# renyi533/euler

Measured on AMD Instinct MI355X. Metric: train samples/sec (whole node), GraphSAGE 2-hop on 100M-node synthetic graph, higher is better.
Workload: dtype bf16; 1 GPU; model=GraphSAGE supervised (2x SAGEConv mean + fc + out_fc, sigmoid CE, Adam), global_batch=1024, parallelism=dp1, num_nodes=100000000, num_edges=950851296, feature_dim=128, feature_dtype=bf16, hidden_dim=256, label_dim=64, hipgraph=True, steps_per_graph=32, impl=euler_amd.models.sage_trainer.SageTrainer (4 fused gfx950 launches per step)

## Files before the change

### euler_amd/_build.py

```python
from __future__ import annotations

import concurrent.futures as cf
import glob
import os
import subprocess
import sys
import sysconfig

ROOT = os.path.dirname(os.path.abspath(__file__))
REPO = os.path.dirname(ROOT)
BUILD = os.environ.get("EULER_AMD_BUILD_DIR", os.path.join(os.path.expanduser("~"), ".cache", "euler_amd_build"))
CSRC = os.path.join(ROOT, "csrc")
ARCH = os.environ.get("EULER_AMD_ARCH", "gfx950")

_EXT_SUFFIX = sysconfig.get_config_var("EXT_SUFFIX") or ".so"


def _log(msg: str) -> None:
    if os.environ.get("EULER_AMD_BUILD_QUIET") != "1":
        print(f"[euler_amd build] {msg}", file=sys.stderr, flush=True)


def _newest(paths) -> float:
    m = 0.0
    for p in paths:
        try:
            m = max(m, os.path.getmtime(p))
        except OSError:
            pass
    return m


def _run(cmd):
    r = subprocess.run(cmd, stdout=subprocess.PIPE, stderr=subprocess.STDOUT, text=True)
    if r.returncode != 0:
        raise RuntimeError("command failed:\n" + " ".join(cmd) + "\n" + r.stdout)
    return r.stdout


def _compile_all(jobs, max_workers):
    todo = []
    for cmd, obj, dep_m, src in jobs:
        if os.path.exists(obj) and os.path.getmtime(obj) >= max(dep_m, os.path.getmtime(src)):
            continue
        todo.append((cmd, obj, src))
    if not todo:
        return False
    with cf.ThreadPoolExecutor(max_workers=max_workers) as ex:
        futs = {ex.submit(_run, cmd): src for cmd, obj, src in todo}
        for f in cf.as_completed(futs):
            f.result()
            _log("compiled " + os.path.relpath(futs[f], REPO))
    return True


def _pybind_includes():
    import pybind11

    return [pybind11.get_include(), sysconfig.get_paths()["include"]]


ENGINE_DIRS = ["common", "graph", "index", "framework", "gql", "ops", "rpc", "pipeline", "bindings"]


def engine_sources():
    srcs = []
    for d in ENGINE_DIRS:
        srcs += sorted(glob.glob(os.path.join(CSRC, d, "*.cc")))
    return srcs


def engine_headers():
    hs = []
    for d in ENGINE_DIRS:
        hs += glob.glob(os.path.join(CSRC, d, "*.h"))
    return hs


def engine_target():
    return os.path.join(ROOT, "_engine" + _EXT_SUFFIX)


def build_engine(max_workers: int = 8, extra_flags=None) -> str:
    out = engine_target()
    objdir = os.path.join(BUILD, "engine")
    os.makedirs(objdir, exist_ok=True)
    flags = ["-O3", "-g1", "-std=c++17", "-fPIC", "-fvisibility=hidden", "-pthread",
             "-fno-omit-frame-pointer", "-Wall", "-Wno-sign-compare", "-Wno-unused-function"]
    flags += list(extra_flags or [])
    inc = ["-I" + CSRC] + ["-I" + p for p in _pybind_includes()]
    hdr_m = _newest(engine_headers() + [__file__])
    if os.path.exists(out) and os.path.getmtime(out) >= max(hdr_m, _newest(engine_sources())):
        return out
    jobs, objs = [], []
    for s in engine_sources():
        rel = os.path.relpath(s, CSRC).replace(os.sep, "_")
        o = os.path.join(objdir, rel + ".o")
        objs.append(o)
        jobs.append((["g++"] + flags + inc + ["-c", s, "-o", o], o, hdr_m, s))
    changed = _compile_all(jobs, max_workers)
    if changed or not os.path.exists(out) or os.path.getmtime(out) < _newest(objs):
        _run(["g++", "-shared", "-pthread", "-o", out] + objs)
        _log("linked " + os.path.relpath(out, REPO))
    return out


def console_target():
    return os.path.join(ROOT, "bin", "remote_console")


def build_console(max_workers: int = 8) -> str:
    build_engine(max_workers)
    out = console_target()
    objdir = os.path.join(BUILD, "engine")
    src = os.path.join(CSRC, "tools", "remote_console.cc")
    flags = ["-O2", "-std=c++17", "-pthread", "-Wall", "-Wno-sign-compare", "-I" + CSRC]
    obj = os.path.join(objdir, "tools_remote_console.cc.o")
    hdr_m = _newest(engine_headers() + [__file__])
    _compile_all([(["g++"] + flags + ["-c", src, "-o", obj], obj, hdr_m, src)], 1)
    objs = []
    for s in engine_sources():
        if os.sep + "bindings" + os.sep in s:
            continue
        o = os.path.join(objdir, os.path.relpath(s, CSRC).replace(os.sep, "_") + ".o")
        if not os.path.exists(o):
            _compile_all([(["g++", "-O3", "-std=c++17", "-fPIC", "-pthread", "-I" + CSRC] +
                           ["-I" + p for p in _pybind_includes()] + ["-c", s, "-o", o], o, hdr_m, s)], 1)
        objs.append(o)
    if not os.path.exists(out) or os.path.getmtime(out) < _newest(objs + [obj]):
        os.makedirs(os.path.dirname(out), exist_ok=True)
        _run(["g++", "-pthread", "-o", out, obj] + objs + ["-ldl"])
        _log("linked " + os.path.relpath(out, REPO))
    return out


_SANITIZERS = {
    "thread": ["-fsanitize=thread"],
    "address": ["-fsanitize=address,undefined", "-fno-sanitize-recover=undefined"],
    "none": [],
}


def build_selftest(sanitize: str = "thread", max_workers: int = 8) -> str:
    if sanitize not in _SANITIZERS:
        raise ValueError("sanitize must be one of %s" % sorted(_SANITIZERS))
    objdir = os.path.join(BUILD, "selftest_" + sanitize)
    os.makedirs(objdir, exist_ok=True)
    out = os.path.join(objdir, "engine_selftest")
    san = _SANITIZERS[sanitize]
    flags = ["-O1", "-g", "-std=c++17", "-pthread", "-fno-omit-frame-pointer", "-Wno-sign-compare"] + san
    srcs = [s for s in engine_sources() if os.sep + "bindings" + os.sep not in s]
    srcs.append(os.path.join(CSRC, "tests", "engine_selftest.cc"))
    hdr_m = _newest(engine_headers() + [__file__])
    jobs, objs = [], []
    for s in srcs:
        rel = os.path.relpath(s, CSRC).replace(os.sep, "_")
        o = os.path.join(objdir, rel + ".o")
        objs.append(o)
        jobs.append((["g++"] + flags + ["-I" + CSRC, "-c", s, "-o", o], o, hdr_m, s))
    changed = _compile_all(jobs, max_workers)
    if changed or not os.path.exists(out) or os.path.getmtime(out) < _newest(objs):
        _run(["g++"] + san + ["-pthread", "-o", out] + objs + ["-ldl"])
        _log("linked " + os.path.relpath(out, REPO))
    return out


def build_plan_selftest() -> str:
    objdir = os.path.join(BUILD, "selftest_address")
    os.makedirs(objdir, exist_ok=True)
    out = os.path.join(objdir, "tree_plan_selftest")
    src = os.path.join(CSRC, "tests", "tree_plan_selftest.cc")
    hdir = os.path.join(CSRC, "hip")
    deps = [src, os.path.join(hdir, "tree_plan.h"), os.path.join(hdir, "tree_args.h"), __file__]
    if not os.path.exists(out) or os.path.getmtime(out) < _newest(deps):
        rocm_inc = os.path.join(os.environ.get("ROCM_PATH", "/opt/rocm"), "include")
        _run(["g++", "-O1", "-g", "-std=c++17", "-fno-omit-frame-pointer", "-Wall"] + _SANITIZERS["address"] +
             ["-D__HIP_PLATFORM_AMD__=1", "-I" + CSRC, "-I" + rocm_inc, src, "-o", out])
        _log("linked " + os.path.relpath(out, REPO))
    return out


def hip_target():
    return os.path.join(ROOT, "_hip_ops" + _EXT_SUFFIX)


def _torch_paths():
    import torch

    tdir = os.path.dirname(torch.__file__)
    inc = [os.path.join(tdir, "include"), os.path.join(tdir, "include", "torch", "csrc", "api", "include")]
    return tdir, inc, os.path.join(tdir, "lib"), bool(torch._C._GLIBCXX_USE_CXX11_ABI)


def build_hip(max_workers: int = 8) -> str:
    hipcc = os.environ.get("HIPCC", "/opt/rocm/bin/hipcc")
    out = hip_target()
    objdir = os.path.join(BUILD, "hip")
    os.makedirs(objdir, exist_ok=True)
    tdir, tinc, tlib, abi = _torch_paths()
    hdir = os.path.join(CSRC, "hip")
    kernels = sorted(glob.glob(os.path.join(hdir, "*.hip")))
    bindings = sorted(glob.glob(os.path.join(hdir, "*.cpp")))
    hdrs = glob.glob(os.path.join(hdir, "*.h")) + [__file__]
    hdr_m = _newest(hdrs)
    if os.path.exists(out) and os.path.getmtime(out) >= max(hdr_m, _newest(kernels + bindings)):
        return out
    kflags = ["-O3", "-std=c++17", "-fPIC", f"--offload-arch={ARCH}", "-munsafe-fp-atomics",
              "-D__HIP_PLATFORM_AMD__=1", "-I" + CSRC, "-Wno-unused-result"]
    kflags += os.environ.get("EULER_AMD_HIP_FLAGS", "").split()
    bflags = ["-O2", "-std=c++17", "-fPIC", "-D__HIP_PLATFORM_AMD__=1", "-DUSE_ROCM=1",
              f"-D_GLIBCXX_USE_CXX11_ABI={int(abi)}", "-DTORCH_API_INCLUDE_EXTENSION_H",
              "-DTORCH_EXTENSION_NAME=_hip_ops", "-I" + CSRC, "-I/opt/rocm/include",
              "-Wno-unused-result", "-Wno-deprecated-declarations"]
    bflags += ["-I" + p for p in tinc + _pybind_includes()]
    jobs, objs = [], []
    for s in kernels:
        o = os.path.join(objdir, os.path.basename(s) + ".o")
        objs.append(o)
        jobs.append(([hipcc] + kflags + ["-c", s, "-o", o], o, hdr_m, s))
    for s in bindings:
        o = os.path.join(objdir, os.path.basename(s) + ".o")
        objs.append(o)
        jobs.append((["g++"] + bflags + ["-c", s, "-o", o], o, hdr_m, s))
    changed = _compile_all(jobs, max_workers)
    if changed or not os.path.exists(out) or os.path.getmtime(out) < _newest(objs):
        link = [hipcc, "-shared", "-fPIC", f"--offload-arch={ARCH}", "-o", out] + objs + [
            "-L" + tlib, "-Wl,-rpath," + tlib, "-lc10", "-lc10_hip", "-ltorch", "-ltorch_cpu",
            "-ltorch_hip", "-ltorch_python", "-lamdhip64"]
        _run(link)
        _log("linked " + os.path.relpath(out, REPO))
    return out


def build_all(max_workers: int = 8) -> None:
    if engine_sources():
        build_engine(max_workers)
        build_console(max_workers)
    build_hip(max_workers)


if __name__ == "__main__":
    what = sys.argv[1:] or ["all"]
    if "all" in what:
        build_all()
    else:
        if "engine" in what:
            build_engine()
        if "hip" in what:
            build_hip()
        if "console" in what:
            build_console()
```

### euler_amd/csrc/hip/binding_tree.cpp

```cpp
#include <cstdio>
#include <cstdlib>

#include "hip/binding_util.h"
#include "hip/tree_plan.h"

using namespace euler_bind;
using namespace euler_hip;

namespace {

bool sync_debug() {
  static const bool on = [] {
    const char* e = std::getenv("EULER_AMD_TREE_SYNC");
    return e && e[0] == '1';
  }();
  return on;
}

void tree_ok(hipError_t e, const char* what) {
  launch_ok(e, what);
  if (sync_debug()) {
    const hipError_t s = hipStreamSynchronize(cur_stream());
    TORCH_CHECK(s == hipSuccess, "euler_amd tree kernel '", what, "' faulted: ", hipGetErrorString(s));
    fprintf(stderr, "[tree-sync] %s ok\n", what);
  }
}

void fill_graph_tree(PlanDict& pd, TrGraph& g, TrTree& tr, int64_t F1, int64_t F2, int64_t logP1, int64_t logP2,
                     uint32_t m1, uint32_t m2) {
  torch::Tensor indptr = pd.T("indptr"), rng = pd.T("rng");
  pd.need(indptr, torch::kInt64, -1, "indptr");
  pd.need(rng, torch::kInt64, 2, "rng");
  const int64_t nt = pd.geti("num_types");
  TORCH_CHECK(nt >= 1 && nt <= 32 && (indptr.numel() - 1) % nt == 0, pd.name(), ": indptr must be [N*T+1]");
  g.indptr = indptr.data_ptr<int64_t>();
  g.num_types = static_cast<int32_t>(nt);
  g.num_rows = (indptr.numel() - 1) / nt;
  torch::Tensor nbr = pd.T("nbr"), cumw = pd.T("cumw"), prob = pd.T("node_prob");
  pd.need(nbr, torch::kInt32, -1, "nbr");
  pd.need(cumw, torch::kFloat32, nbr.numel(), "cumw");
  g.nbr = nbr.data_ptr<int32_t>();
  g.cumw = cumw.data_ptr<float>();
  pd.need(prob, torch::kFloat32, -1, "node_prob");
  g.pop = prob.numel();
  TORCH_CHECK(g.pop > 0, pd.name(), ": empty root population");
  g.prob = prob.data_ptr<float>();
  g.alias = pd.i32("node_alias", g.pop);
  g.root_rows = pd.has("root_rows") ? pd.i32("root_rows", g.pop) : nullptr;
  tr.rng = rng.data_ptr<int64_t>();
  tr.F1 = static_cast<int32_t>(F1);
  tr.F2 = static_cast<int32_t>(F2);
  tr.logP1 = static_cast<int32_t>(logP1);
  tr.logP2 = static_cast<int32_t>(logP2);
  tr.m1 = m1;
  tr.m2 = m2;
}

int plan_route_impl(const PlanDict& pd) {
  const int64_t impl = pd.has("dw_route_impl") ? pd.geti("dw_route_impl") : 2;
  TORCH_CHECK(impl == 0 || impl == 2, pd.name(), ": dw_route_impl must be 0 or 2");
  return static_cast<int>(impl);
}

bool plan_fuse_key(const PlanDict& pd) {
  const int64_t f = pd.has("dw_opt_fuse") ? pd.geti("dw_opt_fuse") : 1;
  TORCH_CHECK(f == 0 || f == 1, pd.name(), ": dw_opt_fuse must be 0 or 1");
  return f == 1;
}

class DwPlan {
 public:
  explicit DwPlan(PlanDict& pd) : pd_(pd), route_impl_(plan_route_impl(pd)), fuse_key_(plan_fuse_key(pd)) {}

  std::vector<TrDwProb> probs;
  TrOptArgs opt{};

  const TrDwProb& add(int64_t P, int64_t Q, int64_t M, const uint16_t* G, const uint16_t* X, const float* dA,
                      const uint32_t* mask, int64_t logPg, int64_t Fg, int64_t self) {
    TORCH_CHECK(M % 32 == 0 && P % 32 == 0 && Q % 32 == 0, pd_.name(), ": dW problem shapes");
    TrDwProb p{};
    p.P = static_cast<int32_t>(P);
    p.Q = static_cast<int32_t>(Q);
    p.MB = static_cast<int32_t>(M / 32);
    if (dA) {
      TORCH_CHECK(tr_plan_routed(p, pd_.has("dw_route_wg") ? pd_.geti("dw_route_wg") : 256), pd_.name(),
                  ": routed dW needs P % 64 == 0 and a positive dw_route_wg");
      p.route = 1;
      p.dA = dA;
      p.mask = mask;
      p.logPg = static_cast<int32_t>(logPg);
      p.Fg = static_cast<int32_t>(Fg);
      p.include_self = static_cast<int32_t>(self);
      p.inv = 1.f / static_cast<float>(Fg + self);
    } else {
      const int64_t target = pd_.has("dw_target_wg") ? pd_.geti("dw_target_wg") : 512;
      const int64_t minkps = pd_.has("dw_min_kps") ? pd_.geti("dw_min_kps") : 4;
      const int64_t fold = pd_.has("dw_fold") ? pd_.geti("dw_fold") : 1;
      TORCH_CHECK(target >= 1 && minkps >= 1 && (fold == 0 || fold == 1), pd_.name(),
                  ": dw_target_wg / dw_min_kps must be positive, dw_fold 0 or 1");
      tr_plan_stored(p, target, minkps, fold == 1);
    }
    p.part = pd_.zeros_ptr<float>(static_cast<int64_t>(p.S) * P * Q, torch::kFloat32);
    p.G = G;
    p.X = X;
    probs.push_back(p);
    return probs.back();
  }

  void add_seg(int64_t off, const TrDwProb& p, const uint16_t* sh, const uint16_t* shT) {
    TrSeg& g = next_seg();
    g.off = off;
    g.n = static_cast<int64_t>(p.P) * p.Q;
    g.part = p.part;
    g.S = p.S;
    g.rows = p.P;
    g.cols = p.Q;
    g.sh = const_cast<uint16_t*>(sh);
    g.shT = const_cast<uint16_t*>(shT);
  }
  void add_vec_seg(int64_t off, int64_t n, const float* part, int64_t S) {
    TrSeg& g = next_seg();
    g.off = off;
    g.n = n;
    g.part = part;
    g.S = static_cast<int32_t>(S);
    g.rows = 1;
  }
  void layout_segs() {
    opt.nblk = tr_seg_layout(opt.seg, opt.nseg, true);
    TORCH_CHECK(opt.nblk >= 1, pd_.name(), ": weight segments need rows % 8, cols % 32");
  }

  void fill_opt(int64_t n, const float* head_part, int64_t nhead, bool rank_stat) {
    torch::Tensor flat = pd_.T("flat");
    pd_.need(flat, torch::kFloat32, -1, "flat");
    const int64_t nbuf = flat.numel();
    TORCH_CHECK(n <= nbuf, pd_.name(), ": offsets must lie inside the flat buffer");
    opt.n = n;
    opt.p = flat.data_ptr<float>();
    opt.g = pd_.f32("grad", nbuf);
    opt.m = pd_.f32("m", nbuf);
    opt.v = pd_.f32("v", nbuf);
    TrOptCore& c = opt.c;
    c.step = pd_.ptr<int64_t>("step", torch::kInt64, 1);
    c.lr = static_cast<float>(pd_.getf("lr"));
    c.b1 = static_cast<float>(pd_.getf("beta1"));
    c.b2 = static_cast<float>(pd_.getf("beta2"));
    c.eps = static_cast<float>(pd_.getf("eps"));
    c.wd = static_cast<float>(pd_.getf("weight_decay"));
    c.grad_scale = 1.f;
    c.kind = static_cast<int32_t>(pd_.geti("opt_kind"));
    c.head_part = head_part;
    c.nhead = static_cast<int32_t>(nhead);
    c.loss_acc = pd_.f32("loss_acc", 1);
    c.loss_out = pd_.f32("loss_out", 1);
    if (rank_stat) c.stat_f = pd_.f32("mrr_sum", 1);
    else c.counts = reinterpret_cast<uint32_t*>(pd_.i32("counts", 3));
  }

  void try_fuse(bool allowed) {
    TrDwGrid grid;
    TrDwLaunch L = launch_of(all(), false, grid);
    if (!fuse_key_ || !allowed || !tr_dw_fuse(L, opt, fopt_)) return;
    sync_ = pd_.zeros(static_cast<int64_t>(fopt_.nsync) * kTrSyncLine, torch::kInt32);
    fopt_.sync = reinterpret_cast<uint32_t*>(sync_.data_ptr<int32_t>());
    fused_ = true;
  }
  bool fused() const { return fused_; }
  int64_t fuse_error() const { return sync_.defined() ? sync_[kTrSyncLine].item<int64_t>() : 0; }

  std::vector<int64_t> all() const {
    std::vector<int64_t> w(probs.size());
    for (size_t i = 0; i < w.size(); ++i) w[i] = static_cast<int64_t>(i);
    return w;
  }

  void launch(const std::vector<int64_t>& which, c10::optional<torch::Tensor> prof, bool fuse, double grad_scale) {
    const c10::DeviceGuard g(pd_.device());
    TrDwGrid grid;
    TrDwLaunch L = launch_of(which, fuse, grid);
    if (fuse) L.opt.c.grad_scale = static_cast<float>(grad_scale);
    if (prof.has_value()) {
      pd_.need(*prof, torch::kInt64, -1, "prof");
      L.prof = reinterpret_cast<long long*>(prof->data_ptr<int64_t>());
    }
    tree_ok(eh_tr_dw(&L, cur_stream()), fuse ? "tr_dw+opt" : "tr_dw");
  }
  int64_t blocks(const std::vector<int64_t>& which, bool fuse) const {
    TrDwGrid grid;
    launch_of(which, fuse, grid);
    return grid.ndw + grid.ntrail;
  }
  std::vector<int64_t> splits() const {
    std::vector<int64_t> s;
    for (const auto& p : probs) s.push_back(p.S);
    return s;
  }
  std::vector<int64_t> folds() const {
    std::vector<int64_t> f;
    for (const auto& p : probs) f.push_back(p.F);
    return f;
  }
  void set_lr(double lr) { opt.c.lr = fopt_.c.lr = static_cast<float>(lr); }
  void set_grad(torch::Tensor g, bool exact) {
    pd_.need(g, torch::kFloat32, exact ? opt.n : -1, "grad");
    TORCH_CHECK(g.numel() >= opt.n, "grad has ", g.numel(), " elements, fewer than the ", opt.n, " parameters");
    grad_ = g;
    opt.g = g.data_ptr<float>();
  }

 private:
  PlanDict& pd_;
  int route_impl_;
  bool fuse_key_, fused_ = false;
  TrDwOpt fopt_{};
  torch::Tensor sync_;
  torch::Tensor grad_;

  TrSeg& next_seg() {
    TORCH_CHECK(opt.nseg < kTrMaxSegs, pd_.name(), ": too many optimizer segments");
    return opt.seg[opt.nseg++] = TrSeg{};
  }

  TrDwLaunch launch_of(const std::vector<int64_t>& which, bool fuse, TrDwGrid& grid) const {
    TrDwLaunch L{};
    L.route_impl = route_impl_;
    bool every = which.size() == probs.size();
    for (size_t k = 0; k < which.size(); ++k) {
      const int64_t i = which[k];
      TORCH_CHECK(i >= 0 && i < (int64_t)probs.size(), "dw: problem index out of range");
      every = every && i == (int64_t)k;
      if (probs[i].route) {
        TORCH_CHECK(L.nroute < 2, "dw: at most two routed problems per launch");
        L.route[L.nroute++] = probs[i];
      } else {
        TORCH_CHECK(L.plain.n < kTrMaxProbs, "dw: too many problems");
        L.plain.p[L.plain.n++] = probs[i];
      }
    }
    if (fuse) {
      TORCH_CHECK(fused_ && every, pd_.name(),
                  ": the optimizer runs in the dW launch of every problem, in the plan's order, of a fused() plan only");
      L.opt = fopt_;
      L.fuse = 1;
    }
    TORCH_CHECK(tr_dw_layout(L, grid), pd_.name(), ": the dW launch is not one the kernel takes");
    return L;
  }
};

class TreePlan : private PlanDict {
 public:
  explicit TreePlan(py::dict d) : PlanDict(d, "TreePlan") {
    L_ = geti("L");
    B_ = geti("B");
    TORCH_CHECK(L_ >= 1 && L_ <= 3, "TreePlan: 1..3 hops");
    TORCH_CHECK(B_ > 0 && B_ % 32 == 0, "TreePlan: batch must be a positive multiple of 32");
    F_ = getv("F");
    logP_ = getv("logP");
    masks_ = getv("masks");
    dims_ = getv("H");
    TORCH_CHECK((int)F_.size() == L_ + 1 && (int)masks_.size() == L_ + 1 && (int)logP_.size() >= L_ &&
                    (int)dims_.size() == L_,
                "TreePlan: F/masks need L+1 entries (index 0 unused), logP L, H L");
    D_ = geti("D");
    E_ = geti("E");
    C_ = geti("C");
    C_real_ = geti("C_real");
    self_ = geti("include_self");
    for (int k = 1; k < L_; ++k) TORCH_CHECK(logP_[k] >= 4 && (1 << logP_[k]) > F_[k], "TreePlan: slot group too small");
    for (int k = 0; k < L_; ++k) TORCH_CHECK(dims_[k] % 64 == 0, "TreePlan: conv widths must be padded to 64");
    TORCH_CHECK(D_ % 16 == 0 && E_ % 32 == 0 && C_ % 32 == 0 && C_real_ <= C_, "TreePlan: padded dims");
    M_.assign(L_, 0);
    M_[0] = B_;
    for (int k = 1; k < L_; ++k) M_[k] = M_[k - 1] << logP_[k];
    fill_graph_tree(*this, graph_, tree_, L_ > 1 ? F_[1] : 0, L_ > 2 ? F_[2] : 0, L_ > 1 ? logP_[1] : 0,
                    L_ > 2 ? logP_[2] : 0, static_cast<uint32_t>(masks_[1]),
                    L_ > 2 ? static_cast<uint32_t>(masks_[2]) : 0u);
    build_fwd();
    build_comb();
    build_head();
    build_dw();
    build_opt();
    dw_.try_fuse(!pipeline_ok());
  }

  bool fused() const { return dw_.fused(); }
  int64_t fuse_error() const { return dw_.fuse_error(); }

  void sample() {
    const c10::DeviceGuard g(device());
    tree_ok(eh_tr_sample(&sample_, cur_stream()), "tr_sample");
  }

  void fwd(c10::optional<torch::Tensor> prof, bool gemm_only) {
    const c10::DeviceGuard g(device());
    TORCH_CHECK(!gemm_only || pipeline_ok(), "TreePlan: no pipelined forward for this plan");
    TrFwdArgs a0 = fwd0_;
    if (prof.has_value()) {
      need(*prof, torch::kInt64, (fwd0_.M / (gemm_only ? 64 : bm0_)) * 8, "prof");
      a0.prof = reinterpret_cast<long long*>(prof->data_ptr<int64_t>());
    }
    tree_ok(eh_tr_fwd(&a0, gemm_only ? 3 : (L_ == 1 ? 1 : 0), feat_fp32_, bm0_, cur_stream()), "tr_fwd");
    if (L_ == 3) tree_ok(eh_tr_fwd(&fwd1_, 2, 0, bm1_, cur_stream()), "tr_fwd(inner)");
  }

  void head(c10::optional<torch::Tensor> prof, bool with_sample) {
    const c10::DeviceGuard g(device());
    TrHeadArgs a = head_;
    if (with_sample) {
      a.smp = sample_;
      a.nsample = static_cast<int32_t>((sample_.M + kTrHeadSampleRows - 1) / kTrHeadSampleRows);
    }
    if (prof.has_value()) {
      need(*prof, torch::kInt64, (B_ / kTrHeadRows) * 8, "prof");
      a.prof = reinterpret_cast<long long*>(prof->data_ptr<int64_t>());
    }
    tree_ok(eh_tr_head(&a, B_, cur_stream()), "tr_head");
  }

  void bwd() {
    if (L_ != 3) return;
    const c10::DeviceGuard g(device());
    tree_ok(eh_tr_bwd(&bwd1_, cur_stream()), "tr_bwd");
  }

  void dw(std::vector<int64_t> which, c10::optional<torch::Tensor> prof, bool fuse, double grad_scale) {
    dw_.launch(which, prof, fuse, grad_scale);
  }
  int64_t dw_blocks(bool fuse) const { return dw_.blocks(dw_.all(), fuse); }

  std::vector<int64_t> problems(bool route) const {
    std::vector<int64_t> out;
    for (size_t i = 0; i < dw_.probs.size(); ++i)
      if (static_cast<bool>(dw_.probs[i].route) == route) out.push_back(static_cast<int64_t>(i));
    return out;
  }

  void opt(int64_t mode, double grad_scale, bool with_sample, bool with_gather) {
    const c10::DeviceGuard g(device());
    TORCH_CHECK(!with_gather || pipeline_ok(), "TreePlan: no pipelined gather for this plan");
    TrOptArgs a = dw_.opt;
    a.c.grad_scale = static_cast<float>(grad_scale);
    if (!with_sample) a.nsample = 0;
    if (with_gather) {
      a.gat = fwd0_;
      a.ngather = static_cast<int32_t>(fwd0_.M / 32);
      a.gat_fp32 = feat_fp32_;
      static const int first = [] {
        const char* e = std::getenv("EULER_AMD_GATHER_FIRST");
        return e ? std::atoi(e) : 1;
      }();
      a.gather_first = first;
      static const int tpb = [] {
        const char* e = std::getenv("EULER_AMD_OPT_TPB");
        return e ? std::atoi(e) : 4;
      }();
      a.opt_tpb = tpb;
    }
    tree_ok(eh_tr_opt(&a, static_cast<int>(mode), cur_stream()), "tr_opt");
  }

  bool pipeline_ok() const {
    return L_ == 2 && fwd0_.a_rows != nullptr && !cached_ && bm0_ <= 64 && logP_[1] <= 5 && D_ % 64 == 0 &&
           fwd0_.M % 64 == 0 && dims_[0] <= 256 &&
           eh_tr_gather32_lds(static_cast<int>(D_), static_cast<int>(fwd0_.FL)) <= 64 * 1024;
  }

  void opt_segments(int64_t mode, std::vector<int64_t> segs, bool head_stats) {
    TORCH_CHECK(mode == 0, "opt_segments: only the reduce (mode 0) runs on a segment subset");
    TORCH_CHECK(!segs.empty() && (int64_t)segs.size() <= dw_.opt.nseg, "opt_segments: bad segment list");
    const c10::DeviceGuard g(device());
    TrOptArgs a = dw_.opt;
    a.nseg = 0;
    for (int64_t k : segs) {
      TORCH_CHECK(k >= 0 && k < dw_.opt.nseg, "opt_segments: segment index out of range");
      a.seg[a.nseg++] = dw_.opt.seg[k];
    }
    a.nblk = tr_seg_layout(a.seg, a.nseg, true);
    a.nsample = 0;
    if (!head_stats) a.c.nhead = 0;
    tree_ok(eh_tr_opt(&a, 0, cur_stream()), "tr_opt(segments)");
  }

  int64_t fwd_blocks() const { return fwd0_.M / bm0_; }
  void set_lr(double lr) { dw_.set_lr(lr); }
  void set_grad(torch::Tensor g) { dw_.set_grad(g, true); }
  void set_grad16(c10::optional<torch::Tensor> g16) {
    if (!g16.has_value()) {
      dw_.opt.g16 = nullptr;
      g16_ = torch::Tensor();
      return;
    }
    need(*g16, torch::kBFloat16, dw_.opt.n, "grad16");
    g16_ = *g16;
    dw_.opt.g16 = reinterpret_cast<uint16_t*>(g16_.data_ptr());
  }
  int64_t num_problems() const { return (int64_t)dw_.probs.size(); }
  int64_t route_blocks(int64_t i) const { return dw_.probs.at(i).route ? dw_.blocks({i}, false) : 0; }
  std::vector<int64_t> splits() const { return dw_.splits(); }
  std::vector<int64_t> folds() const { return dw_.folds(); }

 private:
  int L_, B_, D_, E_, C_, C_real_, self_;
  int feat_fp32_ = 0, bm0_ = 32, bm1_ = 32;
  bool cached_ = false;
  std::vector<int64_t> F_, logP_, masks_, dims_, M_;
  TrGraph graph_{};
  TrTree tree_{};
  TrSampleArgs sample_{};
  TrFwdArgs fwd0_{}, fwd1_{};
  TrHeadArgs head_{};
  TrBwdArgs bwd1_{};
  DwPlan dw_{*this};
  torch::Tensor roots_cur_;
  torch::Tensor g16_;

  int64_t Hin(int k) const { return k == 0 ? D_ : dims_[k - 1]; }

  void build_fwd() {
    const bool cached = has("fwd_features");
    torch::Tensor x = cached ? T("fwd_features") : T("features");
    feat_fp32_ = !need_bf16_or_f32(x, -1, "features");
    TORCH_CHECK(x.dim() == 2 && x.size(1) == D_, "features must be [N, D] with D padded to 16");
    TORCH_CHECK(cached || x.size(0) == graph_.num_rows, "features must have one row per graph row");
    const int lv = L_ - 1;
    const int64_t M = M_[lv];
    TrSampleArgs& sm = sample_;
    sm.g = graph_;
    sm.tr = tree_;
    sm.M = M;
    sm.lv = lv;
    sm.FL = static_cast<int32_t>(F_[L_]);
    sm.mL = static_cast<uint32_t>(masks_[L_]);
    sm.hopL = L_;
    sm.roots = i32("roots", B_);
    sm.nodes = i32("nodes", M);
    sm.leaf = i32("leaf", M * sm.FL);
    TrFwdArgs& a = fwd0_;
    a.x = x.data_ptr();
    a.D = D_;
    a.M = M;
    a.FL = sm.FL;
    a.include_self = self_;
    a.inv_leaf = 1.f / static_cast<float>(a.FL + self_);
    cached_ = cached;
    a.nodes = cached ? i32("fwd_nodes", M) : sm.nodes;
    a.leaf = cached ? i32("fwd_leaf", M * sm.FL) : sm.leaf;
    a.roots_in = sm.roots;
    roots_cur_ = zeros(B_, torch::kInt32);
    a.roots_cur = roots_cur_.data_ptr<int32_t>();
    a.B = B_;
    a.step = ptr<int64_t>("step", torch::kInt64, 1);
    a.rng = ptr<int64_t>("rng", torch::kInt64, 2);
    if (L_ == 1) {
      a.a_next = bf("A0", B_ * 2 * D_);
      bm0_ = 32;
      return;
    }
    a.W = bf("W0_sh", dims_[0] * 2 * D_);
    a.H = static_cast<int32_t>(dims_[0]);
    a.a_kt = bf("A0_kt", M * 2 * D_);
    a.mask = i32_as_u32("mask0", (M / 32) * dims_[0]);
    a.logPg = static_cast<int32_t>(logP_[lv]);
    a.Fg = static_cast<int32_t>(F_[lv]);
    a.inv_grp = 1.f / static_cast<float>(a.Fg + self_);
    a.a_next = bf("A1", M_[lv - 1] * 2 * dims_[0]);
    a.a_rows = has("A0_rows") ? bf("A0_rows", M * 2 * D_) : nullptr;
    bm0_ = (1 << a.logPg) > 32 ? (1 << a.logPg) : 32;
    if (has("fwd_bm")) bm0_ = std::max<int>(bm0_, static_cast<int>(geti("fwd_bm")));
    TORCH_CHECK(bm0_ == 32 || bm0_ == 64 || bm0_ == 128, "TreePlan: fwd rows per block must be 32, 64 or 128");
    TORCH_CHECK(M % bm0_ == 0, "TreePlan: target rows must be a multiple of the fwd block rows");
    if (L_ == 3) {
      TrFwdArgs& b = fwd1_;
      b.x = T("A1").data_ptr();
      b.D = static_cast<int32_t>(dims_[0]);
      b.M = M_[1];
      b.include_self = self_;
      b.W = bf("W1_sh", dims_[1] * 2 * dims_[0]);
      b.H = static_cast<int32_t>(dims_[1]);
      b.a_kt = bf("A1_kt", M_[1] * 2 * dims_[0]);
      b.mask = i32_as_u32("mask1", (M_[1] / 32) * dims_[1]);
      b.logPg = static_cast<int32_t>(logP_[1]);
      b.Fg = static_cast<int32_t>(F_[1]);
      b.inv_grp = 1.f / static_cast<float>(b.Fg + self_);
      b.a_next = bf("A2", B_ * 2 * dims_[1]);
      bm1_ = (1 << b.logPg) > 32 ? (1 << b.logPg) : 32;
    }
  }

  void build_comb() {
    torch::Tensor flat = T("flat");
    need(flat, torch::kFloat32, -1, "flat");
    std::vector<int64_t> off = getv("offsets");
    TORCH_CHECK((int)off.size() == L_ + 4 && off.back() == flat.numel(), "TreePlan: offsets must cover the flat buffer");
    const int64_t H = dims_[L_ - 1];
    TORCH_CHECK(off[L_ + 1] - off[L_] == (int64_t)E_ * H && off[L_ + 3] - off[L_ + 2] == (int64_t)C_ * E_,
                "TreePlan: fc / out_fc segments do not match E, H, C");
    TORCH_CHECK(C_ % 16 == 0 && H % 16 == 0 && E_ % 32 == 0, "TreePlan: combination tiles need C % 16, H % 16, E % 32");
    float* base = flat.data_ptr<float>();
    TrCombArgs& c = fwd0_.comb;
    c.bfc = base + off[L_ + 1];
    c.wout = base + off[L_ + 2];
    c.wout_sh = bf("Wout_sh", (int64_t)C_ * E_);
    c.wfcT_sh = bf("Wfc_shT", (int64_t)E_ * H);
    c.C = C_;
    c.E = E_;
    c.H = static_cast<int32_t>(H);
    c.Wc = zeros_ptr<uint16_t>((int64_t)C_ * H, torch::kBFloat16);
    c.WcT = zeros_ptr<uint16_t>((int64_t)C_ * H, torch::kBFloat16);
    c.bc = zeros_ptr<float>(C_, torch::kFloat32);
    fwd0_.ncomb = 1;
  }

  uint32_t* i32_as_u32(const std::string& k, int64_t numel) { return reinterpret_cast<uint32_t*>(i32(k, numel)); }

  void build_head() {
    const int last = L_ - 1;
    const int64_t Hin2 = 2 * Hin(last), H = dims_[last];
    TrHeadArgs& a = head_;
    a.A = bf("A" + std::to_string(last), B_ * Hin2);
    a.Hin2 = static_cast<int32_t>(Hin2);
    a.H = static_cast<int32_t>(H);
    a.E = E_;
    a.C = C_;
    a.C_real = C_real_;
    a.W = bf("W" + std::to_string(last) + "_sh", H * Hin2);
    a.WT = L_ > 1 ? bf("W" + std::to_string(last) + "_shT", H * Hin2) : nullptr;
    a.Wfc = bf("Wfc_sh", (int64_t)E_ * H);
    a.WfcT = bf("Wfc_shT", (int64_t)E_ * H);
    a.Wout = bf("Wout_sh", (int64_t)C_ * E_);
    a.WoutT = bf("Wout_shT", (int64_t)C_ * E_);
    a.bfc = f32("bfc", E_);
    a.Wc = fwd0_.comb.Wc;
    a.WcT = fwd0_.comb.WcT;
    a.bc = fwd0_.comb.bc;
    a.roots = fwd0_.roots_cur;
    const int mode = static_cast<int>(geti("label_mode"));
    torch::Tensor lab = T("labels");
    need_any(lab, "labels");
    TORCH_CHECK(mode >= 0 && mode <= 2, "label_mode must be 0, 1 or 2");
    const int64_t lrows = has("label_rows") ? geti("label_rows") : graph_.num_rows;
    if (mode == 0) {
      TORCH_CHECK(lab.scalar_type() == torch::kInt16 && lab.numel() == lrows, "TreePlan: labels int16 [N]");
    } else if (mode == 1) {
      TORCH_CHECK(lab.scalar_type() == torch::kInt32 && lab.numel() == lrows, "TreePlan: labels int32 [N]");
    } else {
      TORCH_CHECK(lab.scalar_type() == torch::kBFloat16 && lab.numel() == lrows * C_, "TreePlan: labels bf16 [N, C]");
    }
    a.labels = lab.data_ptr();
    a.label_mode = mode;
    a.inv_scale = 1.f / static_cast<float>(B_ * C_real_);
    a.A_kt = bf("A" + std::to_string(last) + "_kt", B_ * Hin2);
    a.h_kt = bf("h_kt", B_ * H);
    a.emb_kt = bf("emb_kt", (int64_t)B_ * E_);
    a.dlog_kt = bf("dlog_kt", (int64_t)B_ * C_);
    a.demb_kt = bf("demb_kt", (int64_t)B_ * E_);
    a.g_kt = bf("g_kt", B_ * H);
    a.dA = L_ > 1 ? f32("dA" + std::to_string(last), B_ * Hin2) : nullptr;
    const int64_t nblk = B_ / kTrHeadRows;
    a.dbfc_part = zeros_ptr<float>(nblk * E_, torch::kFloat32);
    a.head_part = zeros_ptr<float>(nblk * 4, torch::kFloat32);
    a.prof = nullptr;
    const size_t lds = eh_tr_head_lds(a.Hin2, a.H, a.E, a.C, mode);
    TORCH_CHECK(lds <= 160 * 1024 - 64, "TreePlan: head tile does not fit in LDS (", lds, " bytes)");
    if (L_ == 3) {
      TrBwdArgs& b = bwd1_;
      b.dA = f32("dA2", B_ * 2 * dims_[1]);
      b.mask = i32_as_u32("mask1", (M_[1] / 32) * dims_[1]);
// ... 146 lines not shown
  int bm() const { return bm_; }
  int64_t R() const { return R_; }
  int64_t H() const { return H_; }
  int64_t D() const { return D_; }
  using PlanDict::device;

  void bwd() {
    dw_.launch({0}, c10::nullopt, false, 1.0);
    const c10::DeviceGuard g(device());
    tree_ok(eh_tr_opt(&dw_.opt, 0, cur_stream()), "tower reduce");
  }

 private:
  int64_t R_, F1_, F2_, logP_, D_, H_, self_, M_;
  int feat_fp32_ = 0, bm_ = 32;
  TrGraph g_{};
  TrTree tree_{};
  TrSampleArgs sample_{};
  TrFwdArgs fwd_{};
  DwPlan dw_{*this};

  int32_t* owned_i32(int64_t n) { return full(n, -1, torch::kInt32).data_ptr<int32_t>(); }
};

class PairPlan : private PlanDict {
 public:
  PairPlan(const TowerPlan& s, const TowerPlan& c, py::dict d) : PlanDict(d, "PairPlan", s.device()) {
    B_ = geti("B");
    K_ = geti("K");
    H0_ = s.H();
    H1_ = geti("H1");
    E_ = geti("E");
    TORCH_CHECK(c.R() == B_ * (1 + K_) && s.R() == B_, "PairPlan: tower roots must be B and B (1 + K)");
    TORCH_CHECK(c.H() == H0_ && c.D() == s.D(), "PairPlan: towers must have the same layer-0 shape");
    TORCH_CHECK(B_ % 32 == 0 && K_ >= 1 && K_ <= 15, "PairPlan: B % 32 == 0 and 1 <= K <= 15");
    TORCH_CHECK(H1_ % 64 == 0 && E_ % 32 == 0, "PairPlan: padded dims (H1 % 64, E % 32)");
    TORCH_CHECK(eh_tr_pair_head_lds(static_cast<int>(K_), static_cast<int>(2 * H0_), static_cast<int>(H1_),
                                    static_cast<int>(E_)) <= 160 * 1024 - 256,
                "PairPlan: the pair head does not fit in LDS (K / widths too large)");
    fpx_ = s.feat_fp32();
    bm_s_ = s.bm();
    bm_c_ = c.bm();
    ss_ = s.sample_args();
    sc_ = c.sample_args();
    ss_.tr.root_in = nullptr;
    ss_.tr.root_mode = 0;
    ss_.tr.stream_off = 0;
    sc_.tr.root_in = nullptr;
    sc_.tr.root_mode = 1;
    sc_.tr.pair_B = static_cast<int32_t>(B_);
    sc_.tr.pair_mask = static_cast<uint32_t>(geti("pos_mask"));
    sc_.tr.stream_off = 8;
    fs_ = s.fwd_args();
    fc_ = c.fwd_args();
    fs_.roots_in = ss_.roots;
    fc_.roots_in = sc_.roots;
    fs_.step = ptr<int64_t>("step", torch::kInt64, 1);
    fc_.step = nullptr;
    fc_.rng = zeros_ptr<int64_t>(2, torch::kInt64);
    nblk_ = B_ / 16;
    TrPairHeadArgs& h = head_;
    h.B = static_cast<int32_t>(B_);
    h.K = static_cast<int32_t>(K_);
    h.H0x2 = static_cast<int32_t>(2 * H0_);
    h.H1 = static_cast<int32_t>(H1_);
    h.E = static_cast<int32_t>(E_);
    h.inv_n = 1.f / static_cast<float>(B_ * (1 + K_));
    h.head_part = zeros_ptr<float>(nblk_ * 4, torch::kFloat32);
    tower(h.s, s, "s");
    tower(h.c, c, "c");
    const TowerPlan* tp[2] = {&s, &c};
    const TrPairTower* tw[2] = {&h.s, &h.c};
    for (int t = 0; t < 2; ++t) dw_.probs.push_back(tp[t]->prob());
    for (int t = 0; t < 2; ++t) {
      dw_.add(H1_, 2 * H0_, tp[t]->R(), tw[t]->g_kt, tw[t]->A1_kt, nullptr, nullptr, 0, 0, 0);
      dw_.add(E_, H1_, tp[t]->R(), tw[t]->de_kt, tw[t]->h_kt, nullptr, nullptr, 0, 0, 0);
    }
    std::vector<int64_t> off = getv("offsets");
    TORCH_CHECK(off.size() == 9, "PairPlan: offsets = 8 segments + end");
    for (int t = 0; t < 2; ++t) {
      const TrPairTower& T_ = *tw[t];
      dw_.add_seg(off[4 * t], dw_.probs[t], tp[t]->fwd_args().W, nullptr);
      dw_.add_seg(off[4 * t + 1], dw_.probs[2 + 2 * t], T_.W1, T_.W1T);
      dw_.add_seg(off[4 * t + 2], dw_.probs[3 + 2 * t], T_.Wfc, T_.WfcT);
      dw_.add_vec_seg(off[4 * t + 3], E_, T_.dbfc_part, nblk_);
      TORCH_CHECK(off[4 * t + 4] - off[4 * t + 3] == E_, "PairPlan: bias segment must be E long");
    }
    dw_.layout_segs();
    dw_.fill_opt(off.back(), h.head_part, nblk_, true);
    dw_.try_fuse(true);
  }

  bool fused() const { return dw_.fused(); }
  int64_t fuse_error() const { return dw_.fuse_error(); }

  void sample() {
    const c10::DeviceGuard g(device());
    tree_ok(eh_tr_sample(&ss_, cur_stream()), "pair sample (source)");
    tree_ok(eh_tr_sample(&sc_, cur_stream()), "pair sample (context)");
  }
  void fwd() {
    const c10::DeviceGuard g(device());
    tree_ok(eh_tr_fwd(&fs_, 0, fpx_, bm_s_, cur_stream()), "pair fwd (source)");
    tree_ok(eh_tr_fwd(&fc_, 0, fpx_, bm_c_, cur_stream()), "pair fwd (context)");
  }
  void head() {
    const c10::DeviceGuard g(device());
    tree_ok(eh_tr_pair_head(&head_, cur_stream()), "pair head");
  }
  void dw(bool fuse, double grad_scale) { dw_.launch(dw_.all(), c10::nullopt, fuse, grad_scale); }
  void opt(int mode, double grad_scale) {
    const c10::DeviceGuard g(device());
    TrOptArgs a = dw_.opt;
    a.c.grad_scale = static_cast<float>(grad_scale);
    tree_ok(eh_tr_opt(&a, mode, cur_stream()), "pair opt");
  }
  void set_lr(double lr) { dw_.set_lr(lr); }
  void set_grad(torch::Tensor g) { dw_.set_grad(g, false); }
  std::vector<int64_t> splits() const { return dw_.splits(); }
  std::vector<int64_t> folds() const { return dw_.folds(); }

 private:
  int64_t B_, K_, H0_, H1_, E_, nblk_;
  int fpx_ = 0, bm_s_ = 32, bm_c_ = 32;
  TrSampleArgs ss_{}, sc_{};
  TrFwdArgs fs_{}, fc_{};
  TrPairHeadArgs head_{};
  DwPlan dw_{*this};

  void tower(TrPairTower& t, const TowerPlan& tp, const std::string& x) {
    const int64_t R = tp.R();
    t.A1 = tp.fwd_args().a_next;
    t.W1 = bf(("W1_sh_" + x).c_str(), H1_ * 2 * H0_);
    t.W1T = bf(("W1_shT_" + x).c_str(), H1_ * 2 * H0_);
    t.Wfc = bf(("Wfc_sh_" + x).c_str(), E_ * H1_);
    t.WfcT = bf(("Wfc_shT_" + x).c_str(), E_ * H1_);
    t.bfc = ptr<float>(("bfc_" + x).c_str(), torch::kFloat32, E_);
    t.A1_kt = zeros_ptr<uint16_t>(R * 2 * H0_, torch::kBFloat16);
    t.h_kt = zeros_ptr<uint16_t>(R * H1_, torch::kBFloat16);
    t.de_kt = zeros_ptr<uint16_t>(R * E_, torch::kBFloat16);
    t.g_kt = zeros_ptr<uint16_t>(R * H1_, torch::kBFloat16);
    t.dA1 = const_cast<float*>(tp.prob().dA);
    t.dbfc_part = zeros_ptr<float>(nblk_ * E_, torch::kFloat32);
  }
};

}

void register_tree_ops(py::module& m) {
  static_assert(kTrHeadSampleRows == 256, "head sampler blocks: 1024 threads, 256 rows");
  py::class_<TreePlan>(m, "TreePlan")
      .def(py::init<py::dict>())
      .def("sample", &TreePlan::sample)
      .def("fwd", &TreePlan::fwd, py::arg("prof") = py::none(), py::arg("gemm_only") = false)
      .def("fwd_blocks", [](const TreePlan& t) { return t.fwd_blocks(); })
      .def("head", &TreePlan::head, py::arg("prof") = py::none(), py::arg("with_sample") = false)
      .def("bwd", &TreePlan::bwd)
      .def("dw", &TreePlan::dw, py::arg("which"), py::arg("prof") = py::none(), py::arg("fuse") = false,
           py::arg("grad_scale") = 1.0)
      .def("fused", &TreePlan::fused)
      .def("dw_blocks", &TreePlan::dw_blocks, py::arg("fuse"))
      .def("fuse_error", &TreePlan::fuse_error)
      .def("route_blocks", &TreePlan::route_blocks)
      .def("opt", &TreePlan::opt, py::arg("mode"), py::arg("grad_scale") = 1.0, py::arg("with_sample") = false,
           py::arg("with_gather") = false)
      .def("pipeline_ok", &TreePlan::pipeline_ok)
      .def("opt_segments", &TreePlan::opt_segments, py::arg("mode"), py::arg("segs"), py::arg("head_stats"))
      .def("set_lr", &TreePlan::set_lr)
      .def("set_grad16", &TreePlan::set_grad16, py::arg("g16"))
      .def("set_grad", &TreePlan::set_grad, py::arg("g"))
      .def("num_problems", &TreePlan::num_problems)
      .def("splits", &TreePlan::splits)
      .def("folds", &TreePlan::folds)
      .def("problems", &TreePlan::problems, py::arg("route"));
  m.attr("tree_head_rows") = kTrHeadRows;
  py::class_<TowerPlan>(m, "TowerPlan")
      .def(py::init<py::dict>())
      .def("shadow", &TowerPlan::shadow)
      .def("sample", &TowerPlan::sample)
      .def("fwd", &TowerPlan::fwd)
      .def("bwd", &TowerPlan::bwd)
      .def("fused", &TowerPlan::fused)
      .def("fuse_error", &TowerPlan::fuse_error);
  py::class_<PairPlan>(m, "PairPlan")
      .def(py::init<const TowerPlan&, const TowerPlan&, py::dict>(), py::keep_alive<1, 2>(), py::keep_alive<1, 3>())
      .def("sample", &PairPlan::sample)
      .def("fwd", &PairPlan::fwd)
      .def("head", &PairPlan::head)
      .def("dw", &PairPlan::dw, py::arg("fuse") = false, py::arg("grad_scale") = 1.0)
      .def("fused", &PairPlan::fused)
      .def("fuse_error", &PairPlan::fuse_error)
      .def("opt", &PairPlan::opt, py::arg("mode"), py::arg("grad_scale") = 1.0)
      .def("set_lr", &PairPlan::set_lr)
      .def("set_grad", &PairPlan::set_grad)
      .def("splits", &PairPlan::splits)
      .def("folds", &PairPlan::folds);
}
```

### euler_amd/csrc/hip/tree_args.h

```cpp
#pragma once
#include <hip/hip_runtime_api.h>
#include <stdint.h>

namespace euler_hip {

constexpr int kTrMaxProbs = 6;
constexpr int kTrMaxSegs = 8;
constexpr int kTrHeadRows = 16;
constexpr int kTrHeadSampleRows = 256;

struct TrGraph {
  const int64_t* indptr;
  const int32_t* nbr;
  const float* cumw;
  int64_t num_rows;
  int32_t num_types;
  const float* prob;
  const int32_t* alias;
  const int32_t* root_rows;
  int64_t pop;
};

struct TrTree {
  const int64_t* rng;
  const int32_t* root_in;
  int32_t F1, F2;
  int32_t logP1, logP2;
  uint32_t m1, m2;
  int32_t root_mode, pair_B;
  uint32_t pair_mask;
  int32_t stream_off;
};

struct TrSampleArgs {
  TrGraph g;
  TrTree tr;
  int64_t M;
  int32_t lv;
  int32_t FL;
  uint32_t mL;
  int32_t hopL;
  int32_t* roots;
  int32_t* nodes;
  int32_t* leaf;
};

struct TrCombArgs {
  const float* wout;
  const float* bfc;
  const uint16_t* wout_sh;
  const uint16_t* wfcT_sh;
  int32_t C, E, H;
  uint16_t* Wc;
  uint16_t* WcT;
  float* bc;
};

struct TrFwdArgs {
  const void* x;
  int32_t D;
  int64_t M;
  int32_t FL;
  int32_t include_self;
  float inv_leaf;
  const int32_t* nodes;
  const int32_t* leaf;
  const uint16_t* W;
  int32_t H;
  uint16_t* a_kt;
  uint32_t* mask;
  uint16_t* a_next;
  int32_t logPg, Fg;
  float inv_grp;
  int64_t* step;
  int64_t* rng;
  const int32_t* roots_in;
  int32_t* roots_cur;
  int32_t B;
  long long* prof;
  TrCombArgs comb;
  int32_t ncomb;
  uint16_t* a_rows;
};

struct TrHeadArgs {
  const uint16_t* A;
  int32_t Hin2, H, E, C, C_real;
  const uint16_t *W, *WT, *Wfc, *WfcT, *Wout, *WoutT;
  const uint16_t *Wc, *WcT;
  const float* bfc;
  const float* bc;
  const int32_t* roots;
  const void* labels;
  int32_t label_mode;
  float inv_scale;
  uint16_t *A_kt, *h_kt, *emb_kt, *dlog_kt, *demb_kt, *g_kt;
  float* dA;
  float* dbfc_part;
  float* head_part;
  long long* prof;
  TrSampleArgs smp;
  int32_t nsample;
};

struct TrPairTower {
  const uint16_t* A1;
  const uint16_t *W1, *W1T;
  const uint16_t *Wfc, *WfcT;
  const float* bfc;
  uint16_t *A1_kt, *h_kt, *de_kt, *g_kt;
  float* dA1;
  float* dbfc_part;
};
struct TrPairHeadArgs {
  TrPairTower s, c;
  int32_t B, K, H0x2, H1, E;
  float inv_n;
  float* head_part;
};

struct TrBwdArgs {
  const float* dA;
  const uint32_t* mask;
  const uint16_t* WT;
  int32_t Hk, K2out;
  int64_t M;
  int32_t logPg, Fg, include_self;
  float inv;
  float* dA_out;
};

struct TrDwProb {
  const uint16_t* G;
  const uint16_t* X;
  float* part;
  int32_t P, Q, MB, kps, S, tiles_q, ntiles, wg0;
  int32_t F;
  const float* dA;
  const uint32_t* mask;
  int32_t route, logPg, Fg, include_self;
  float inv;
};
struct TrDwProbs {
  TrDwProb p[kTrMaxProbs];
  int32_t n;
};
constexpr int kTrFoldLds = 64 * 1024;
constexpr int kTrFoldMax = kTrFoldLds / (32 * 32 * 4);

struct TrSeg {
  int64_t off, n;
  const float* part;
  int32_t S;
  int32_t rows, cols;
  int32_t blk0;
  uint16_t* sh;
  uint16_t* shT;
  int32_t sgrp;
};
struct TrOptCore {
  const int64_t* step;
  float lr, b1, b2, eps, wd, grad_scale;
  int32_t kind;
  const float* head_part;
  int32_t nhead;
  float* loss_acc;
  uint32_t* counts;
  float* loss_out;
  float* stat_f;
};
struct TrOptArgs {
  float *p, *g, *m, *v;
  uint16_t* g16;
  int64_t n;
  TrSeg seg[kTrMaxSegs];
  int32_t nseg;
  int32_t nblk;
  TrOptCore c;
  TrSampleArgs smp;
  int32_t nsample;
  TrFwdArgs gat;
  int32_t ngather;
  int32_t gat_fp32;
  int32_t gather_first;
  int32_t opt_tpb;
};

struct TrFoldSeg {
  int64_t off;
  uint16_t *sh, *shT;
};
struct TrDwOpt {
  float *p, *m, *v;
  TrSeg seg[kTrMaxSegs];
  int32_t nseg, nblk;
  int32_t rseg0;
  TrFoldSeg fseg[kTrMaxProbs];
  TrOptCore c;
  uint32_t* sync;
  int32_t nsync;
  int32_t cnt0[2];
  long long timeout;
};
constexpr int kTrSyncLine = 32;
constexpr uint32_t kTrFuseTimeout = 1u;
constexpr long long kTrFuseWaitTicks = 1200000;

struct TrDwLaunch {
  TrDwProbs plain;
  TrDwProb route[2];
  int32_t nroute;
  int32_t rwg[3];
  int32_t route_impl;
  long long* prof;
  int32_t ndw;
  int32_t fuse;
  TrDwOpt opt;
};

}

extern "C" {
hipError_t eh_tr_sample(const euler_hip::TrSampleArgs* a, hipStream_t s);
hipError_t eh_tr_fwd(const euler_hip::TrFwdArgs* a, int mode, int feat_fp32, int bm, hipStream_t s);
size_t eh_tr_gather32_lds(int D, int FL);
hipError_t eh_tr_head(const euler_hip::TrHeadArgs* a, int64_t B, hipStream_t s);
hipError_t eh_tr_bwd(const euler_hip::TrBwdArgs* a, hipStream_t s);
hipError_t eh_tr_dw(euler_hip::TrDwLaunch* p, hipStream_t s);
hipError_t eh_tr_opt(const euler_hip::TrOptArgs* a, int mode, hipStream_t s);
size_t eh_tr_fwd_lds(int D, int H, int bm, int FL, int mode);
size_t eh_tr_fwd2_lds(int D, int FL);
size_t eh_tr_head_lds(int Hin2, int H, int E, int C, int label_mode);
size_t eh_tr_pair_head_lds(int K, int H0x2, int H1, int E);
hipError_t eh_tr_pair_head(const euler_hip::TrPairHeadArgs* a, hipStream_t s);
}
```

### euler_amd/csrc/hip/tree_dev.h

```cpp
#pragma once
#include "hip/tile.h"
#include "hip/tree_args.h"

namespace euler_hip {

constexpr uint64_t kTrStreamRoot = 1, kTrStreamPos = 2, kTrStreamNeg = 3, kTrStreamHop = 16;

#define TR_STAMP(prof, blk, k) \
  if ((prof) && threadIdx.x == 0) (prof)[(blk) * 8 + (k)] = static_cast<long long>(wall_clock64())

__device__ __forceinline__ uint4_t tr_rand(const int64_t* rng, uint64_t stream, uint64_t idx) {
  return Philox::gen(static_cast<uint64_t>(rng[0]), (static_cast<uint64_t>(rng[1]) << 8) ^ stream, idx);
}

__device__ __forceinline__ int32_t tr_root(const TrGraph& g, const int64_t* rng, int64_t t,
                                           uint64_t stream = kTrStreamRoot) {
  const uint4_t r = tr_rand(rng, stream, static_cast<uint64_t>(t));
  const uint64_t x = (static_cast<uint64_t>(r[0]) << 32) | r[1];
  int64_t k = static_cast<int64_t>(__umul64hi(x, static_cast<uint64_t>(g.pop)));
  if (k >= g.pop) k = g.pop - 1;
  const int64_t pick = (u01(r[2]) < g.prob[k]) ? k : static_cast<int64_t>(g.alias[k]);
  return g.root_rows ? g.root_rows[pick] : static_cast<int32_t>(pick);
}

// ... 2 lines not shown
  const int64_t base = static_cast<int64_t>(row) * g.num_types;
  int64_t lo = 0, hi = 0;
  float total = 0.f;
  if (g.num_types == 1) {
    if (!(mask & 1u)) return -1;
    lo = g.indptr[base];
    hi = g.indptr[base + 1];
    total = hi > lo ? g.cumw[hi - 1] : 0.f;
  } else {
    float tot = 0.f;
    for (int t = 0; t < g.num_types; ++t) {
      if (!((mask >> t) & 1u)) continue;
      const int64_t a = g.indptr[base + t], b = g.indptr[base + t + 1];
      if (b > a) tot += g.cumw[b - 1];
    }
    if (!(tot > 0.f)) return -1;
    float u = u01(r[0]) * tot;
    for (int t = 0; t < g.num_types; ++t) {
      if (!((mask >> t) & 1u)) continue;
      const int64_t a = g.indptr[base + t], b = g.indptr[base + t + 1];
      if (b <= a) continue;
      const float gw = g.cumw[b - 1];
      lo = a;
      hi = b;
      total = gw;
      if (u < gw) break;
      u -= gw;
    }
  }
  if (hi <= lo || !(total > 0.f)) return -1;
  const float u = u01(r[1]) * total;
  int64_t a = lo, b = hi - 1;
  while (a < b) {
    const int64_t m = (a + b) >> 1;
    if (g.cumw[m] > u) b = m;
    else a = m + 1;
  }
  return g.nbr[a];
}

__device__ __forceinline__ int32_t tr_hop(const TrGraph& g, const int64_t* rng, int32_t parent, int j, int F,
                                          uint32_t mask, int hop, int64_t parent_slot, int stream_off = 0) {
  if (j < F)
    return parent >= 0 ? tr_neighbor(g, parent, mask,
                                     tr_rand(rng, kTrStreamHop + hop + stream_off,
                                             static_cast<uint64_t>(parent_slot * F + j)))
                       : -1;
  return j == F ? parent : -1;
}

__device__ __forceinline__ int32_t tr_tree_root(const TrGraph& g, const TrTree& tr, int64_t t) {
  if (tr.root_in) return tr.root_in[t];
  if (tr.root_mode == 0) return tr_root(g, tr.rng, t);
  if (t < tr.pair_B) {
    const int32_t src = tr_root(g, tr.rng, t);
    return src >= 0 ? tr_neighbor(g, src, tr.pair_mask, tr_rand(tr.rng, kTrStreamPos, static_cast<uint64_t>(t)))
                    : -1;
  }
  return tr_root(g, tr.rng, t, kTrStreamNeg);
}

__device__ int32_t tr_slot_node(const TrGraph& g, const TrTree& tr, int64_t s, int lv, int64_t* root,
                                bool* self_chain) {
  int64_t i0 = s, i1 = 0, i2 = 0;
  if (lv == 1) {
    i1 = s;
    i0 = s >> tr.logP1;
  } else if (lv == 2) {
    i2 = s;
    i1 = s >> tr.logP2;
    i0 = i1 >> tr.logP1;
  }
  int32_t node = tr_tree_root(g, tr, i0);
  bool sc = true;
  if (lv >= 1) {
    const int j = static_cast<int>(i1 & ((int64_t(1) << tr.logP1) - 1));
    sc = j == tr.F1;
    node = tr_hop(g, tr.rng, node, j, tr.F1, tr.m1, 1, i0, tr.stream_off);
  }
  if (lv >= 2) {
    const int j = static_cast<int>(i2 & ((int64_t(1) << tr.logP2) - 1));
    sc = sc && j == tr.F2;
    node = tr_hop(g, tr.rng, node, j, tr.F2, tr.m2, 2, i1, tr.stream_off);
  }
  *root = i0;
  *self_chain = sc;
  return node;
}

__device__ __forceinline__ float bf_lo(uint32_t v) { return __uint_as_float(v << 16); }
__device__ __forceinline__ float bf_hi(uint32_t v) { return __uint_as_float(v & 0xffff0000u); }

template <typename FT>
struct Feat8;
template <>
struct Feat8<bf16_t> {
  static constexpr int kInFlight = 10;
  uint4_t v;
  __device__ __forceinline__ void load(const bf16_t* p) { v = *reinterpret_cast<const uint4_t*>(p); }
  __device__ __forceinline__ void zero() { v = uint4_t{0u, 0u, 0u, 0u}; }
  __device__ __forceinline__ void add_to(float* acc) const { acc_bf16x8(acc, v); }
  __device__ __forceinline__ void add_scaled_to(float* acc, float w) const {
#pragma unroll
    for (int i = 0; i < 4; ++i) {
      acc[2 * i] += w * bf_lo(v[i]);
      acc[2 * i + 1] += w * bf_hi(v[i]);
    }
  }
  __device__ __forceinline__ void keep(bool k) {
#pragma unroll
    for (int i = 0; i < 4; ++i) v[i] = k ? v[i] : 0u;
  }
  __device__ __forceinline__ uint4_t bf16() const { return v; }
};
template <>
struct Feat8<float> {
  static constexpr int kInFlight = 5;
  float4_t a, b;
  __device__ __forceinline__ void load(const float* p) {
    a = *reinterpret_cast<const float4_t*>(p);
    b = *reinterpret_cast<const float4_t*>(p + 4);
  }
  __device__ __forceinline__ void zero() { a = b = float4_t{0.f, 0.f, 0.f, 0.f}; }
  __device__ __forceinline__ void add_to(float* acc) const {
#pragma unroll
    for (int i = 0; i < 4; ++i) {
      acc[i] += a[i];
      acc[4 + i] += b[i];
    }
  }
  __device__ __forceinline__ void add_scaled_to(float* acc, float w) const {
#pragma unroll
    for (int i = 0; i < 4; ++i) {
      acc[i] += w * a[i];
      acc[4 + i] += w * b[i];
    }
  }
  __device__ __forceinline__ void keep(bool k) {
#pragma unroll
    for (int i = 0; i < 4; ++i) {
      a[i] = k ? a[i] : 0.f;
      b[i] = k ? b[i] : 0.f;
    }
  }
  __device__ __forceinline__ uint4_t bf16() const {
    float t[8] = {a[0], a[1], a[2], a[3], b[0], b[1], b[2], b[3]};
    return pack_bf16x8(t);
  }
};

constexpr int kTrSampleRows = 64;

template <int NT>
__device__ __forceinline__ void tr_sample_block(const TrSampleArgs& a, int blk, int32_t* node_s) {
  constexpr int R = NT / 4;
  const int64_t row0 = static_cast<int64_t>(blk) * R;
  if (threadIdx.x < R) {
    const int64_t s = row0 + threadIdx.x;
    int32_t node = -1;
    if (s < a.M) {
      int64_t root;
      bool sc;
      node = tr_slot_node(a.g, a.tr, s, a.lv, &root, &sc);
      if (sc) a.roots[root] = node;
      a.nodes[s] = node;
    }
    node_s[threadIdx.x] = node;
  }
  __syncthreads();
  for (int it = threadIdx.x; it < R * a.FL; it += NT) {
    const int r = it / a.FL, k = it - r * a.FL;
    const int64_t s = row0 + r;
    if (s >= a.M) break;
    const int32_t node = node_s[r];
    a.leaf[s * a.FL + k] =
        node >= 0 ? tr_neighbor(a.g, node, a.mL,
                                tr_rand(a.tr.rng, kTrStreamHop + a.hopL + a.tr.stream_off,
                                        static_cast<uint64_t>(s * a.FL + k)))
                  : -1;
  }
}

#ifndef F2_SKIP_PAD
#define F2_SKIP_PAD 1
#endif

__device__ __forceinline__ int f2_chunk(int r, int c) { return c ^ (r & 15); }

template <typename FT, int BM, int NT>
__device__ __forceinline__ void f2_gather(const TrFwdArgs& a, bf16_t* At, const int32_t* node_s,
                                          const int32_t* leaf_s, int tid) {
  const int D = a.D, K2 = 2 * D;
  const FT* x = static_cast<const FT*>(a.x);
  const int cpr = D >> 3;
  const int P = 1 << a.logPg, U = F2_SKIP_PAD ? a.Fg + 1 : P;
  const int nitems = (BM >> a.logPg) * U * cpr;
  constexpr int G = Feat8<FT>::kInFlight;
  if (F2_SKIP_PAD && U < P) {
    const int pad = P - U, nch = K2 >> 3;
    for (int it = tid; it < (BM >> a.logPg) * pad * nch; it += NT) {
      const int q = it / nch, c = it - q * nch;
      const int r = (q / pad) * P + U + q % pad;
      *reinterpret_cast<uint4_t*>(At + r * K2 + f2_chunk(r, c) * 8) = uint4_t{0u, 0u, 0u, 0u};
    }
  }
  for (int it = tid; it < nitems; it += 2 * NT) {
    const int itb = it + NT;
    const bool hb = itb < nitems;
    const int qa = it / cpr, ca = it - qa * cpr;
    const int qb = hb ? itb / cpr : qa, cb = hb ? itb - qb * cpr : ca;
    const int ra = (qa / U) * P + qa % U, rb = (qb / U) * P + qb % U;
    const int32_t na = node_s[ra], nb = hb ? node_s[rb] : -1;
    Feat8<FT> sa, sb;
    float acc_a[8], acc_b[8];
#pragma unroll
    for (int i = 0; i < 8; ++i) acc_a[i] = acc_b[i] = 0.f;
    sa.load(x + static_cast<int64_t>(na > 0 ? na : 0) * D + ca * 8);
    sb.load(x + static_cast<int64_t>(nb > 0 ? nb : 0) * D + cb * 8);
    for (int k = 0; k < a.FL; k += G) {
      int32_t ja[G], jb[G];
      Feat8<FT> va[G], vb[G];
#pragma unroll
      for (int u = 0; u < G; ++u) {
        ja[u] = (k + u < a.FL) ? leaf_s[ra * a.FL + k + u] : -1;
        jb[u] = (hb && k + u < a.FL) ? leaf_s[rb * a.FL + k + u] : -1;
      }
#pragma unroll
      for (int u = 0; u < G; ++u) {
        va[u].load(x + static_cast<int64_t>(ja[u] > 0 ? ja[u] : 0) * D + ca * 8);
        vb[u].load(x + static_cast<int64_t>(jb[u] > 0 ? jb[u] : 0) * D + cb * 8);
      }
#pragma unroll
      for (int u = 0; u < G; ++u) {
        va[u].keep(ja[u] >= 0);
        vb[u].keep(jb[u] >= 0);
        va[u].add_to(acc_a);
        vb[u].add_to(acc_b);
      }
    }
    sa.keep(na >= 0);
    sb.keep(nb >= 0);
    if (a.include_self) {
      sa.add_to(acc_a);
      sb.add_to(acc_b);
    }
#pragma unroll
    for (int i = 0; i < 8; ++i) {
      acc_a[i] *= a.inv_leaf;
      acc_b[i] *= a.inv_leaf;
    }
#pragma unroll
    for (int h = 0; h < 2; ++h) {
      if (h == 1 && !hb) break;
      const int r = h ? rb : ra, c = h ? cb : ca;
      *reinterpret_cast<uint4_t*>(At + r * K2 + f2_chunk(r, c) * 8) = h ? sb.bf16() : sa.bf16();
      *reinterpret_cast<uint4_t*>(At + r * K2 + f2_chunk(r, cpr + c) * 8) = pack_bf16x8(h ? acc_b : acc_a);
    }
  }
}

template <int BM, int NT>
__device__ __forceinline__ void f2_kt(const TrFwdArgs& a, int64_t row0, const bf16_t* At, int tid) {
  const int K2 = 2 * a.D;
  const int np = K2 >> 1;
  for (int it = tid; it < np * (BM / 8); it += NT) {
    const int q = it / np;
    const int n = (it - q * np) * 2;
    uint32_t w[8];
#pragma unroll
    for (int i = 0; i < 8; ++i) {
      const int r = q * 8 + i;
      w[i] = *reinterpret_cast<const uint32_t*>(At + r * K2 + f2_chunk(r, n >> 3) * 8 + (n & 7));
    }
    uint4_t lo, hi;
    kt_pack8(w, lo, hi);
    *reinterpret_cast<uint4_t*>(a.a_kt + kt_off(row0 + q * 8, n, K2)) = lo;
    *reinterpret_cast<uint4_t*>(a.a_kt + kt_off(row0 + q * 8, n + 1, K2)) = hi;
  }
}

constexpr int kG32Rows = 32, kG32Threads = 256;

template <typename FT>
__device__ __forceinline__ void tr_gather32_tile(const TrFwdArgs& a, int tile, bf16_t* lds) {
  constexpr int BM = kG32Rows, NT = kG32Threads;
  const int K2 = 2 * a.D, tid = threadIdx.x;
  const int64_t row0 = static_cast<int64_t>(tile) * BM;
  bf16_t* At = lds;
  int32_t* node_s = reinterpret_cast<int32_t*>(lds + BM * K2);
  int32_t* leaf_s = node_s + BM;
  if (tid < BM) node_s[tid] = a.nodes[row0 + tid];
  for (int it = tid; it < BM * a.FL; it += NT) leaf_s[it] = a.leaf[row0 * a.FL + it];
  __syncthreads();
  f2_gather<FT, BM, NT>(a, At, node_s, leaf_s, tid);
  __syncthreads();
  f2_kt<BM, NT>(a, row0, At, tid);
  const int cpr2 = K2 >> 3;
  for (int it = tid; it < BM * cpr2; it += NT) {
    const int r = it / cpr2, c = it - r * cpr2;
    *reinterpret_cast<uint4_t*>(a.a_rows + (row0 + r) * K2 + c * 8) =
        *reinterpret_cast<const uint4_t*>(At + r * K2 + f2_chunk(r, c) * 8);
  }
}

}
```

### euler_amd/csrc/hip/tree_dw.hip

```cpp
#include "hip/tree_dev.h"
#include "hip/tree_plan.h"

namespace euler_hip {

struct RouteRaw {
  uint32_t bits;
  float ds, dn;
};

__device__ __forceinline__ RouteRaw tr_route_load(const TrDwProb& pr, int mb, int p, int lk) {
  const int64_t m0 = static_cast<int64_t>(mb) * 32 + lk;
  const float* row = pr.dA + (m0 >> pr.logPg) * 2 * pr.P;
  RouteRaw r;
  r.bits = pr.mask[static_cast<int64_t>(mb) * pr.P + p] >> lk;
  r.ds = row[p];
  r.dn = row[pr.P + p];
  return r;
}

__device__ __forceinline__ uint4_t tr_route_frag(const TrDwProb& pr, const RouteRaw& r, int mb, int lk) {
  const int j0 = static_cast<int>((static_cast<int64_t>(mb) * 32 + lk) & ((int64_t(1) << pr.logPg) - 1));
  const float dn = r.dn * pr.inv;
  const float ds = r.ds + (pr.include_self ? dn : 0.f);
  float v[8];
// ... 494 lines not shown
    mw[j] = mj;
    vw[j] = vj;
  }
  *reinterpret_cast<float4_t*>(o.p + fi) = pw;
  *reinterpret_cast<float4_t*>(o.m + fi) = mw;
  *reinterpret_cast<float4_t*>(o.v + fi) = vw;
  if (!fz.sh) return;
  __syncthreads();
  float(*st)[33] = reinterpret_cast<float(*)[33]>(slots);
#pragma unroll
  for (int j = 0; j < 4; ++j) st[row][c4 + j] = pw[j];
  __syncthreads();
  tr_opt_shadow(fz.sh, fz.shT, pr.P, pr.Q, p0 + wave * 8, q0, st + wave * 8, lane);
}

__device__ __forceinline__ void tr_fuse_wait(const TrDwOpt& a, const uint32_t* cnt, uint32_t want) {
  if (threadIdx.x == 0) {
    const long long t0 = wall_clock64();
    while (__hip_atomic_load(cnt, __ATOMIC_RELAXED, __HIP_MEMORY_SCOPE_AGENT) != want) {
      if (wall_clock64() - t0 > a.timeout) {
        __hip_atomic_store(a.sync + kTrSyncLine, kTrFuseTimeout, __ATOMIC_RELAXED, __HIP_MEMORY_SCOPE_AGENT);
        __hip_atomic_store(a.c.loss_out, __builtin_nanf(""), __ATOMIC_RELAXED, __HIP_MEMORY_SCOPE_AGENT);
        break;
      }
      __builtin_amdgcn_s_sleep(8);
    }
    __builtin_amdgcn_fence(__ATOMIC_ACQUIRE, "agent");
    asm volatile("s_waitcnt vmcnt(0)" ::: "memory");
  }
  __syncthreads();
}

template <bool FUSE>
__device__ __forceinline__ float tr_slab_load(const float* p) {
  if constexpr (FUSE) return __hip_atomic_load(p, __ATOMIC_RELAXED, __HIP_MEMORY_SCOPE_AGENT);
  else return *p;
}

template <int MODE, bool FUSE = false, class A = TrOptArgs>
__device__ __forceinline__ void tr_opt_tile(const A& a, int b, float (*tile_s)[33]) {
  static_assert(!FUSE || MODE == 2, "trailing blocks run the fused reduce + update");
  const int tid = threadIdx.x;
  if (b == 0 && tid < 64 && MODE != 3 && a.c.nhead > 0) {
    if constexpr (MODE != 1) {
      float v[4] = {0.f, 0.f, 0.f, 0.f};
      for (int k = tid; k < a.c.nhead; k += 64)
#pragma unroll
        for (int c = 0; c < 4; ++c) v[c] += a.c.head_part[k * 4 + c];
#pragma unroll
      for (int c = 0; c < 4; ++c) v[c] = wave_sum(v[c]);
      if (tid == 0) {
        a.c.loss_acc[0] = v[0];
        if (a.c.stat_f) {
          a.c.stat_f[0] += v[1];
        } else if (a.c.counts) {
          a.c.counts[0] += static_cast<uint32_t>(v[1]);
          a.c.counts[1] += static_cast<uint32_t>(v[2]);
          a.c.counts[2] += static_cast<uint32_t>(v[3]);
        }
        if (MODE == 2) a.c.loss_out[0] = v[0];
      }
    } else if (tid == 0) {
      a.c.loss_out[0] = a.c.loss_acc[0];
    }
  }
  TrSeg sg = a.seg[0];
  int ks = 0;
#pragma unroll
  for (int k = 1; k < kTrMaxSegs; ++k)
    if (k < a.nseg && b >= a.seg[k].blk0) {
      sg = a.seg[k];
      ks = k;
    }
  (void)ks;
  const int local = b - sg.blk0;
  int64_t i;
  int r = 0, c = 0;
  bool valid = true;
  const int grp = sg.cols == 0 && sg.sgrp > 1 ? sg.sgrp : 1;
  const int per = 256 / grp, sub = tid / per;
  if (sg.cols > 0) {
    const int tiles_c = sg.cols >> 5;
    const int tr = local / tiles_c, tc = local - tr * tiles_c;
    r = tr * 8 + (tid >> 5);
    c = tc * 32 + (tid & 31);
    i = sg.off + static_cast<int64_t>(r) * sg.cols + c;
  } else {
    i = sg.off + static_cast<int64_t>(local) * per + (tid - sub * per);
    valid = i < sg.off + sg.n;
    if (!valid) i = sg.off;
    valid = valid && sub == 0;
  }
  float p = a.p[i];
  float m = 0.f, v = 0.f;
  if (MODE == 1 || MODE == 2) {
    m = a.m[i];
    v = a.v[i];
  }
  if constexpr (FUSE) {
    if (ks >= a.rseg0) {
      const int rt = (r >> 6) * ((sg.cols + 127) >> 7) + (c >> 7);
      const int c0 = ks == a.rseg0 ? a.cnt0[0] : a.cnt0[1];
      tr_fuse_wait(a, a.sync + static_cast<int64_t>(c0 + rt) * kTrSyncLine, static_cast<uint32_t>(sg.S));
    }
  }
  if (MODE != 3) {
    float g;
    if constexpr (MODE != 1) {
      const float* src = sg.part + (i - sg.off);
      g = 0.f;
      if (sg.S == 1) g += tr_slab_load<FUSE>(src);
      for (int s0 = sub; sg.S > 1 && s0 < sg.S; s0 += 16 * grp) {
        float v[16];
#pragma unroll
        for (int u = 0; u < 16; ++u) {
          const int sl = s0 + u * grp;
          v[u] = tr_slab_load<FUSE>(src + static_cast<int64_t>(sl < sg.S ? sl : sg.S - 1) * sg.n);
        }
#pragma unroll
        for (int u = 0; u < 16; ++u) g += (s0 + u * grp < sg.S) ? v[u] : 0.f;
      }
      if (grp > 1) {
        float* red = &tile_s[0][0];
        red[tid] = g;
        __syncthreads();
        const int e = tid - sub * per;
        g = red[e];
        for (int q = 1; q < grp; ++q) g += red[q * per + e];
      }
      if constexpr (MODE == 0) {
        if (valid) {
          if (a.g16) a.g16[i] = f2bf(g);
          else a.g[i] = g;
        }
        return;
      }
    } else {
      g = a.g16 ? bf2f(a.g16[i]) : a.g[i];
    }
    tr_opt_update(a.c, g, p, m, v);
    if (valid) {
      a.p[i] = p;
      a.m[i] = m;
      a.v[i] = v;
    }
  }
  if (sg.cols > 0 && sg.sh) {
    tile_s[tid >> 5][tid & 31] = p;
    __syncthreads();
    if (tid < 64) tr_opt_shadow(sg.sh, sg.shT, sg.rows, sg.cols, r - (tid >> 5), c - (tid & 31), tile_s, tid);
  }
}

__global__ __launch_bounds__(256, 2) void tr_dw_all_kernel(TrDwLaunch a) {
  __shared__ __attribute__((aligned(16))) RouteLds gs;
  __shared__ uint4_t lut[256];
  const int b = blockIdx.x;
  const bool pipe = a.route_impl == 2;
  if (!pipe && a.nroute > 0 && b < a.rwg[a.nroute]) {
    tr_spread_lut_init(lut);
    __syncthreads();
  }
  if (pipe && a.nroute > 0 && b < a.rwg[a.nroute]) {
    const bool second = b >= a.rwg[1];
    TrDwProb pr = a.route[0];
    if (second) pr = a.route[1];
    uint32_t* ready = a.fuse ? a.opt.sync + static_cast<int64_t>(second ? a.opt.cnt0[1] : a.opt.cnt0[0]) * kTrSyncLine : nullptr;
    tr_dw_route_pipe_body(pr, second ? b - a.rwg[1] : b, gs, lut, second ? nullptr : a.prof, ready);
  } else if (a.nroute > 0 && b < a.rwg[1]) {
    tr_dw_route_body(a.route[0], b, gs, lut, a.prof,
                     a.fuse ? a.opt.sync + static_cast<int64_t>(a.opt.cnt0[0]) * kTrSyncLine : nullptr);
  } else if (a.nroute > 1 && b < a.rwg[2]) {
    tr_dw_route_body(a.route[1], b - a.rwg[1], gs, lut, nullptr,
                     a.fuse ? a.opt.sync + static_cast<int64_t>(a.opt.cnt0[1]) * kTrSyncLine : nullptr);
  } else if (b < a.ndw) {
    const int r = a.rwg[a.nroute];
    const int id = xcd_remap(b - r, a.ndw - r);
    TrDwProb pr = a.plain.p[0];
    TrFoldSeg fz = a.opt.fseg[0];
#pragma unroll
    for (int i = 1; i < kTrMaxProbs; ++i)
      if (a.plain.n > i && id >= a.plain.p[i].wg0) {
        pr = a.plain.p[i];
        fz = a.opt.fseg[i];
      }
    float* slots = reinterpret_cast<float*>(&gs[0][0][0]);
    if (pr.F > 0) tr_dw_fold_body(pr, id - pr.wg0, slots, a.opt, fz, a.fuse != 0);
    else tr_dw_plain_body(pr, id - pr.wg0);
  } else {
    tr_opt_tile<2, true>(a.opt, b - a.ndw, reinterpret_cast<float(*)[33]>(&gs[0][0][0]));
    if (threadIdx.x == 0) {
      const uint32_t nt = static_cast<uint32_t>(gridDim.x) - static_cast<uint32_t>(a.ndw);
      if (__hip_atomic_fetch_add(a.opt.sync, 1u, __ATOMIC_RELAXED, __HIP_MEMORY_SCOPE_AGENT) == nt - 1u) {
        for (int k = 2; k < a.opt.nsync; ++k)
          __hip_atomic_store(a.opt.sync + static_cast<int64_t>(k) * kTrSyncLine, 0u, __ATOMIC_RELAXED,
                             __HIP_MEMORY_SCOPE_AGENT);
        __hip_atomic_store(a.opt.sync, 0u, __ATOMIC_RELAXED, __HIP_MEMORY_SCOPE_AGENT);
      }
    }
  }
}

template <int MODE, typename FT, int GATHER>
__global__ __launch_bounds__(256, GATHER ? 4 : 1) void tr_opt_kernel(TrOptArgs a) {
  __shared__ float tile_s[8][33];
  __shared__ int32_t node_s[kTrSampleRows];
  extern __shared__ __attribute__((aligned(16))) bf16_t glds[];
  int b = blockIdx.x;
  const int tpb = GATHER && a.opt_tpb > 1 ? a.opt_tpb : 1;
  const int nopt = (a.nblk + tpb - 1) / tpb;
  if constexpr (GATHER) {
    if (a.gather_first) {
      if (b < a.ngather) {
        tr_gather32_tile<FT>(a.gat, b, glds);
        return;
      }
      b -= a.ngather;
    } else if (b >= nopt + a.nsample) {
      tr_gather32_tile<FT>(a.gat, b - nopt - a.nsample, glds);
      return;
    }
  }
  if (b >= nopt) {
    tr_sample_block<256>(a.smp, b - nopt, node_s);
    return;
  }
  for (int r = 0; r < tpb; ++r) {
    const int bt = b * tpb + r;
    if (bt >= a.nblk) break;
    tr_opt_tile<MODE>(a, bt, tile_s);
    if (tpb > 1) __syncthreads();
  }
}

}

using namespace euler_hip;

extern "C" {

static_assert(kRP == kTrRouteP && kRQ == kTrRouteQ, "tree_plan.h plans the routed tiles of tr_dw_route");

hipError_t eh_tr_dw(TrDwLaunch* L, hipStream_t s) {
  TrDwGrid grid;
  if (!tr_dw_layout(*L, grid)) return hipErrorInvalidValue;
  if (grid.ndw == 0) return hipSuccess;
  hipLaunchKernelGGL(tr_dw_all_kernel, dim3(static_cast<uint32_t>(grid.ndw + grid.ntrail)), dim3(256), 0, s, *L);
  return hipGetLastError();
}

size_t eh_tr_gather32_lds(int D, int FL) {
  return static_cast<size_t>(kG32Rows) * 2 * D * sizeof(bf16_t) + static_cast<size_t>(kG32Rows) * (1 + FL) * sizeof(int32_t);
}

hipError_t eh_tr_opt(const TrOptArgs* ain, int mode, hipStream_t s) {
  TrOptArgs A = *ain;
  const TrOptArgs* a = &A;
  if (!(mode == 1 || mode == 2)) A.nsample = 0;
  if (mode == 3) A.ngather = 0;
  if (!a->p || !a->g || !a->m || !a->v || !a->c.step || !a->c.loss_acc || !a->c.loss_out || !a->c.head_part ||
      a->c.nhead < 0 || (a->c.nhead == 0 && mode != 0 && mode != 3))
    return hipErrorInvalidValue;
  if (a->nblk < 1 || tr_seg_layout(A.seg, a->nseg, false) != a->nblk) return hipErrorInvalidValue;
  int extra = 0;
  if (a->nsample > 0) {
    if (!tr_sample_ok(a->smp, kTrSampleRows, a->nsample)) return hipErrorInvalidValue;
    extra = a->nsample;
  }
  size_t lds = 0;
  if (a->ngather > 0) {
    const TrFwdArgs& g = a->gat;
    if (!g.x || !g.nodes || !g.leaf || !g.a_kt || !g.a_rows || g.FL < 1 || g.D % 8 != 0 || g.D <= 0 ||
        g.M % kG32Rows != 0 || a->ngather != g.M / kG32Rows || g.logPg < 2 || (1 << g.logPg) > kG32Rows ||
        g.Fg >= (1 << g.logPg))
      return hipErrorInvalidValue;
    lds = eh_tr_gather32_lds(g.D, g.FL);
    if (lds > 64 * 1024) return hipErrorInvalidValue;
    extra += a->ngather;
  }
  const int tpb = a->ngather > 0 && a->opt_tpb > 1 ? a->opt_tpb : 1;
  const int nopt = (a->nblk + tpb - 1) / tpb;
  const dim3 grid(static_cast<uint32_t>(nopt + extra));
#define TR_OPT(MODEV, FT, G) hipLaunchKernelGGL((tr_opt_kernel<MODEV, FT, G>), grid, dim3(256), lds, s, A)
  if (a->ngather > 0 && a->gat_fp32) {
    if (mode == 0) TR_OPT(0, float, 1);
    else if (mode == 1) TR_OPT(1, float, 1);
    else if (mode == 2) TR_OPT(2, float, 1);
    else return hipErrorInvalidValue;
  } else if (a->ngather > 0) {
    if (mode == 0) TR_OPT(0, bf16_t, 1);
    else if (mode == 1) TR_OPT(1, bf16_t, 1);
    else if (mode == 2) TR_OPT(2, bf16_t, 1);
    else return hipErrorInvalidValue;
  } else {
    if (mode == 0) TR_OPT(0, bf16_t, 0);
    else if (mode == 1) TR_OPT(1, bf16_t, 0);
    else if (mode == 2) TR_OPT(2, bf16_t, 0);
    else if (mode == 3) TR_OPT(3, bf16_t, 0);
    else return hipErrorInvalidValue;
  }
#undef TR_OPT
  return hipGetLastError();
}

}
```

### euler_amd/csrc/hip/tree_fwd.hip

```cpp
#include <cstdlib>

#include "hip/tree_dev.h"
#include "hip/tree_plan.h"

namespace euler_hip {

constexpr int kTrBN = 256;

__device__ __forceinline__ void tr_comb_wave(const TrCombArgs& c, int first, int stride, int lane) {
  const int tcols = c.H >> 4, ntiles = (c.C >> 4) * tcols;
  for (int t = first; t < ntiles; t += stride) {
    const int c0 = (t / tcols) * 16, h0 = (t % tcols) * 16;
    float4_t acc = float4_t{0.f, 0.f, 0.f, 0.f};
    for (int k0 = 0; k0 < c.E; k0 += 128) {
      uint4_t av[4], bv[4];
#pragma unroll
      for (int s = 0; s < 4; ++s) {
        const int k = k0 + s * 32 < c.E ? k0 + s * 32 : 0;
        av[s] = fm_frag(c.wout_sh, c0, k, c.E, lane);
        bv[s] = fm_frag(c.wfcT_sh, h0, k, c.E, lane);
      }
#pragma unroll
      for (int s = 0; s < 4; ++s)
        if (k0 + s * 32 < c.E) acc = mfma16(av[s], bv[s], acc);
// ... 141 lines not shown
  }
  if constexpr (MODE != 1) {
    if (wave * 64 < a.H) {
#pragma unroll
      for (int q = 0; q < kBP; ++q)
#pragma unroll
        for (int n = 0; n < FN; ++n) bq[q][n] = fm_frag(W, wave * 64 + n * 16, q * 32 < K2 ? q * 32 : 0, K2, lane);
    }
  }
  __syncthreads();
  TR_STAMP(a.prof, tb, 2);

  if (a.a_kt) {
    constexpr int CH = BM / 8;
    const int np = K2 >> 1;
    for (int it = threadIdx.x; it < np * CH; it += 256) {
      const int q = it / np;
      const int n = (it - q * np) * 2;
      const int64_t gr = row0 + q * 8;
      if (gr >= a.M) continue;
      uint32_t w[8];
#pragma unroll
      for (int i = 0; i < 8; ++i) w[i] = *reinterpret_cast<const uint32_t*>(lds + (q * 8 + i) * ldsw + n);
      uint4_t lo, hi;
      kt_pack8(w, lo, hi);
      *reinterpret_cast<uint4_t*>(a.a_kt + kt_off(gr, n, K2)) = lo;
      *reinterpret_cast<uint4_t*>(a.a_kt + kt_off(gr, n + 1, K2)) = hi;
    }
  }

  TR_STAMP(a.prof, tb, 3);
  constexpr int FM = BM / 16;
  const int lr = lane & 15, lk = (lane >> 4) * 8;
  const int ldo = kTrBN + 8;
  for (int cchunk = 0; cchunk < H; cchunk += kTrBN) {
    const int cb = cchunk + wave * 64;
    float4_t acc[FM][FN];
    tl_zero(acc);
    if (cb < H) {
      if (cchunk > 0) {
#pragma unroll
        for (int q = 0; q < kBP; ++q)
#pragma unroll
          for (int n = 0; n < FN; ++n) bq[q][n] = fm_frag(W, cb + n * 16, q * 32 < K2 ? q * 32 : 0, K2, lane);
      }
      for (int k0 = 0; k0 < K2; k0 += 32 * kBP) {
#pragma unroll
        for (int q = 0; q < kBP; ++q) {
          const int ks = k0 + 32 * q;
          if (ks >= K2) break;
          uint4_t av[FM];
#pragma unroll
          for (int m = 0; m < FM; ++m)
            av[m] = *reinterpret_cast<const uint4_t*>(lds + (m * 16 + lr) * ldsw + ks + lk);
#pragma unroll
          for (int m = 0; m < FM; ++m)
#pragma unroll
            for (int n = 0; n < FN; ++n) acc[m][n] = mfma16(av[m], bq[q][n], acc[m][n]);
          const int kn = ks + 32 * kBP;
#pragma unroll
          for (int n = 0; n < FN; ++n) bq[q][n] = fm_frag(W, cb + n * 16, kn < K2 ? kn : 0, K2, lane);
        }
      }
    }
    if (alias_out) __syncthreads();
    if (cb < H) {
#pragma unroll
      for (int m = 0; m < FM; ++m)
#pragma unroll
        for (int n = 0; n < FN; ++n)
#pragma unroll
          for (int j = 0; j < 4; ++j) {
            const int row = m * 16 + (lane >> 4) * 4 + j;
            otile[row * ldo + wave * 64 + n * 16 + lr] = f2bf(fmaxf(acc[m][n][j], 0.f));
          }
    }
    __syncthreads();
    TR_STAMP(a.prof, tb, 4);
    const int ncols = (H - cchunk) < kTrBN ? (H - cchunk) : kTrBN;
    {
      const int groups = BM >> a.logPg;
      const int pairs = ncols >> 1;
      for (int it = threadIdx.x; it < groups * pairs; it += 256) {
        const int gi = it / pairs;
        const int c = (it - gi * pairs) * 2;
        const int base = gi << a.logPg;
        if (row0 + base >= a.M) continue;
        const uint32_t selfp = *reinterpret_cast<const uint32_t*>(otile + (base + a.Fg) * ldo + c);
        float s0 = 0.f, s1 = 0.f;
        for (int j = 0; j < a.Fg; ++j) {
          const uint32_t v = *reinterpret_cast<const uint32_t*>(otile + (base + j) * ldo + c);
          s0 += bf_lo(v);
          s1 += bf_hi(v);
        }
        if (a.include_self) {
          s0 += bf_lo(selfp);
          s1 += bf_hi(selfp);
        }
        const int64_t parent = (row0 >> a.logPg) + gi;
        bf16_t* dst = a.a_next + parent * 2 * H + cchunk + c;
        *reinterpret_cast<uint32_t*>(dst) = selfp;
        *reinterpret_cast<uint32_t*>(dst + H) = pack_bf16x2(s0 * a.inv_grp, s1 * a.inv_grp);
      }
    }
    if (a.mask) {
      constexpr int KBB = BM / 32;
      for (int it = threadIdx.x; it < KBB * ncols; it += 256) {
        const int kbl = it / ncols, n = it - kbl * ncols;
        const int64_t gr = row0 + kbl * 32;
        if (gr >= a.M) continue;
        uint32_t bits = 0;
#pragma unroll
        for (int i = 0; i < 32; ++i) bits |= (bf_pos(otile[(kbl * 32 + i) * ldo + n]) ? 1u : 0u) << i;
        a.mask[(gr >> 5) * H + cchunk + n] = bits;
      }
    }
    __syncthreads();
  }
  TR_STAMP(a.prof, tb, 5);
}

constexpr int kF2Rows = 64, kF2Threads = 512, kF2Ldt = kF2Rows + 4;
#ifndef F2_ALIAS
#define F2_ALIAS 1
#endif
#ifndef F2_WPF
#define F2_WPF 4
#endif

template <typename FT, int GO>
__global__ __launch_bounds__(kF2Threads, 4) void tr_fwd2_kernel(TrFwdArgs a) {
  extern __shared__ __attribute__((aligned(16))) bf16_t lds[];
  constexpr int BM = kF2Rows, NT = kF2Threads;
  const int tb = static_cast<int>(blockIdx.x), ntb = static_cast<int>(gridDim.x);
  const int D = a.D, K2 = 2 * D, H = a.H;
  const int tile = xcd_remap(tb, ntb);
  const int64_t row0 = static_cast<int64_t>(tile) * BM;
  bf16_t* At = lds;
#if F2_ALIAS
  bf16_t* Ot = lds;
  int32_t* node_s = reinterpret_cast<int32_t*>(lds + (BM * K2 > kTrBN * kF2Ldt ? BM * K2 : kTrBN * kF2Ldt));
#else
  bf16_t* Ot = lds + BM * K2;
  int32_t* node_s = reinterpret_cast<int32_t*>(Ot + kTrBN * kF2Ldt);
#endif
  int32_t* leaf_s = node_s + BM;
  TR_STAMP(a.prof, tb, 0);
  if (a.prof && threadIdx.x == 0) a.prof[tb * 8 + 6] = static_cast<long long>(__smid());
  const int tid = threadIdx.x, wave = tid >> 6, lane = tid & 63;
  const int lr = lane & 15, lg = lane >> 4;
  if (tb == 0 && tid == 0) {
    if (a.step) a.step[0] += 1;
    a.rng[1] += 1;
  }
  for (int i = tb * NT + tid; i < a.B; i += ntb * NT) a.roots_cur[i] = a.roots_in[i];
  if constexpr (GO) {
    const int cpr2 = K2 >> 3;
    for (int it = tid; it < BM * cpr2; it += NT) {
      const int r = it / cpr2, c = it - r * cpr2;
      *reinterpret_cast<uint4_t*>(At + r * K2 + f2_chunk(r, c) * 8) =
          *reinterpret_cast<const uint4_t*>(a.a_rows + (row0 + r) * K2 + c * 8);
    }
  } else {
    if (tid < BM) node_s[tid] = a.nodes[row0 + tid];
    for (int it = tid; it < BM * a.FL; it += NT) leaf_s[it] = a.leaf[row0 * a.FL + it];
    __syncthreads();
  }
  TR_STAMP(a.prof, tb, 1);
  if constexpr (!GO) f2_gather<FT, BM, NT>(a, At, node_s, leaf_s, tid);
  if (a.ncomb && wave == 0) tr_comb_wave(a.comb, tb, ntb, lane);
  const bf16_t* W = a.W;
  constexpr int WPF = F2_WPF;
  uint4_t bq[WPF][2];
  if (wave * 32 < H) {
#pragma unroll
    for (int q = 0; q < WPF; ++q)
#pragma unroll
      for (int n = 0; n < 2; ++n) bq[q][n] = fm_frag(W, wave * 32 + n * 16, q * 32 < K2 ? q * 32 : 0, K2, lane);
  }
  __syncthreads();
  TR_STAMP(a.prof, tb, 2);
  if constexpr (!GO) f2_kt<BM, NT>(a, row0, At, tid);
  TR_STAMP(a.prof, tb, 3);
  constexpr int FM = BM / 16, FN = 2;
  for (int cchunk = 0; cchunk < H; cchunk += kTrBN) {
    const int cb = cchunk + wave * 32;
    float4_t acc[FM][FN];
    tl_zero(acc);
    if (cb < H) {
      if (cchunk > 0) {
#pragma unroll
        for (int q = 0; q < WPF; ++q)
#pragma unroll
          for (int n = 0; n < FN; ++n) bq[q][n] = fm_frag(W, cb + n * 16, q * 32 < K2 ? q * 32 : 0, K2, lane);
      }
      for (int k0 = 0; k0 < K2; k0 += 32 * WPF) {
#pragma unroll
        for (int q = 0; q < WPF; ++q) {
          const int ks = k0 + 32 * q;
          if (ks >= K2) break;
          uint4_t av[FM];
          const int phys = f2_chunk(lr, (ks >> 3) + lg) * 8;
#pragma unroll
          for (int m = 0; m < FM; ++m) av[m] = *reinterpret_cast<const uint4_t*>(At + (m * 16 + lr) * K2 + phys);
#pragma unroll
          for (int m = 0; m < FM; ++m)
#pragma unroll
            for (int n = 0; n < FN; ++n) acc[m][n] = mfma16(av[m], bq[q][n], acc[m][n]);
          const int kn = ks + 32 * WPF;
#pragma unroll
          for (int n = 0; n < FN; ++n) bq[q][n] = fm_frag(W, cb + n * 16, kn < K2 ? kn : 0, K2, lane);
        }
      }
    }
#if F2_ALIAS
    __syncthreads();
#endif
    if (cb < H) {
#pragma unroll
      for (int m = 0; m < FM; ++m)
#pragma unroll
        for (int n = 0; n < FN; ++n) {
          tl_uint2 v;
          v[0] = pack_bf16x2(fmaxf(acc[m][n][0], 0.f), fmaxf(acc[m][n][1], 0.f));
          v[1] = pack_bf16x2(fmaxf(acc[m][n][2], 0.f), fmaxf(acc[m][n][3], 0.f));
          *reinterpret_cast<tl_uint2*>(Ot + (wave * 32 + n * 16 + lr) * kF2Ldt + m * 16 + lg * 4) = v;
        }
    }
    __syncthreads();
    TR_STAMP(a.prof, tb, 4);
    const int ncols = (H - cchunk) < kTrBN ? (H - cchunk) : kTrBN;
    {
      const int P = 1 << a.logPg;
      const int groups = BM >> a.logPg;
      for (int it = tid; it < groups * ncols; it += NT) {
        const int gi = it / ncols, c = it - gi * ncols;
        const bf16_t* col = Ot + c * kF2Ldt + (gi << a.logPg);
        float s = 0.f, self = 0.f;
        for (int r4 = 0; r4 < P; r4 += 4) {
          const tl_uint2 v = *reinterpret_cast<const tl_uint2*>(col + r4);
          const float e[4] = {bf_lo(v[0]), bf_hi(v[0]), bf_lo(v[1]), bf_hi(v[1])};
#pragma unroll
          for (int j = 0; j < 4; ++j) {
            const int r = r4 + j;
            s += r < a.Fg ? e[j] : 0.f;
            self = r == a.Fg ? e[j] : self;
          }
        }
        if (a.include_self) s += self;
        const int64_t parent = (row0 >> a.logPg) + gi;
        bf16_t* dst = a.a_next + parent * 2 * H + cchunk + c;
        dst[0] = f2bf(self);
        dst[H] = f2bf(s * a.inv_grp);
      }
    }
    if (a.mask) {
      for (int it = tid; it < (BM / 32) * ncols; it += NT) {
        const int kbl = it / ncols, c = it - kbl * ncols;
        const bf16_t* col = Ot + c * kF2Ldt + kbl * 32;
        uint32_t bits = 0;
#pragma unroll
        for (int r4 = 0; r4 < 32; r4 += 4) {
          const tl_uint2 v = *reinterpret_cast<const tl_uint2*>(col + r4);
          bits |= (bf_pos(static_cast<bf16_t>(v[0] & 0xffffu)) ? 1u : 0u) << r4;
          bits |= (bf_pos(static_cast<bf16_t>(v[0] >> 16)) ? 1u : 0u) << (r4 + 1);
          bits |= (bf_pos(static_cast<bf16_t>(v[1] & 0xffffu)) ? 1u : 0u) << (r4 + 2);
          bits |= (bf_pos(static_cast<bf16_t>(v[1] >> 16)) ? 1u : 0u) << (r4 + 3);
        }
        a.mask[((row0 >> 5) + kbl) * H + cchunk + c] = bits;
      }
    }
    __syncthreads();
  }
  TR_STAMP(a.prof, tb, 5);
}

__global__ __launch_bounds__(256) void tr_bwd_kernel(TrBwdArgs a) {
  extern __shared__ __attribute__((aligned(16))) bf16_t lds[];
  constexpr int BM = 32;
  const int Hk = a.Hk, K2 = a.K2out;
  const int ldg = Hk + 8;
  const int64_t row0 = static_cast<int64_t>(xcd_remap(blockIdx.x, gridDim.x)) * BM;
  const int Pm = (1 << a.logPg) - 1;
  for (int it = threadIdx.x; it < BM * Hk; it += 256) {
    const int r = it / Hk, n = it - r * Hk;
    const int64_t row = row0 + r;
    float v = 0.f;
    if (row < a.M && ((a.mask[(row >> 5) * Hk + n] >> (row & 31)) & 1u)) {
      const int64_t t = row >> a.logPg;
      const int j = static_cast<int>(row & Pm);
      const float dn = a.dA[t * 2 * Hk + Hk + n] * a.inv;
      if (j < a.Fg) v = dn;
      else if (j == a.Fg) v = a.dA[t * 2 * Hk + n] + (a.include_self ? dn : 0.f);
    }
    lds[r * ldg + n] = f2bf(v);
  }
  __syncthreads();
  const int wave = threadIdx.x >> 6, lane = threadIdx.x & 63;
  const int lr = lane & 15, lk = (lane >> 4) * 8;
  constexpr int FM = BM / 16, FN = 4;
  for (int cchunk = 0; cchunk < K2; cchunk += kTrBN) {
    const int cb = cchunk + wave * 64;
    if (cb >= K2) continue;
    float4_t acc[FM][FN];
    tl_zero(acc);
    for (int k0 = 0; k0 < Hk; k0 += 32) {
// ... 130 lines not shown
```

### euler_amd/csrc/hip/tree_head.hip

```cpp
#include <algorithm>

#include "hip/tree_dev.h"
#include "hip/tree_plan.h"

namespace euler_hip {

constexpr int HB = kTrHeadRows;
constexpr int HFM = HB / 16;
constexpr int HNW = 16;
constexpr int TR_KC = 8;

__device__ __forceinline__ int sw_off(int r, int col, int ld) { return r * ld + col; }

__device__ __forceinline__ void tr_prefetch(const bf16_t* __restrict__ Bf, int col0, int N, int K, int lane,
                                            uint4_t (&b)[TR_KC]) {
  const int c = col0 < N ? col0 : 0;
#pragma unroll
  for (int s = 0; s < TR_KC; ++s) b[s] = fm_frag(Bf, c, s * 32 < K ? s * 32 : 0, K, lane);
}

__device__ __forceinline__ void tr_mfma_chunk(const bf16_t* A, int lda, int kc, int K, const uint4_t (&b)[TR_KC],
                                              float4_t (&acc)[HFM][1], int lane) {
  const int lr = lane & 15, lk = (lane >> 4) * 8;
#pragma unroll
  for (int s = 0; s < TR_KC; ++s) {
    if (kc + s * 32 < K) {
      uint4_t av[HFM];
#pragma unroll
      for (int m = 0; m < HFM; ++m) av[m] = *reinterpret_cast<const uint4_t*>(A + sw_off(m * 16 + lr, kc + s * 32 + lk, lda));
#pragma unroll
      for (int m = 0; m < HFM; ++m) acc[m][0] = mfma16(av[m], b[s], acc[m][0]);
    }
  }
}

__device__ __forceinline__ void tr_gemm(const bf16_t* A, int lda, const bf16_t* __restrict__ Bf, int col0, int K,
                                        float4_t (&acc)[HFM][1], int lane, const uint4_t (&pre)[TR_KC]) {
  tr_mfma_chunk(A, lda, 0, K, pre, acc, lane);
  for (int kc = 32 * TR_KC; kc < K; kc += 32 * TR_KC) {
    uint4_t b[TR_KC];
#pragma unroll
    for (int s = 0; s < TR_KC; ++s) b[s] = fm_frag(Bf, col0, kc + s * 32 < K ? kc + s * 32 : 0, K, lane);
    tr_mfma_chunk(A, lda, kc, K, b, acc, lane);
  }
}

__device__ __forceinline__ void tr_lds_to_kt(const bf16_t* tile, int ld, int N, int64_t r0, bf16_t* kt) {
  const int np = N >> 1;
  for (int it = threadIdx.x; it < np * (HB / 8); it += HNW * 64) {
    const int q = it / np, n = (it - q * np) * 2;
    uint32_t w[8];
#pragma unroll
    for (int i = 0; i < 8; ++i) w[i] = *reinterpret_cast<const uint32_t*>(tile + sw_off(q * 8 + i, n, ld));
    uint4_t lo, hi;
    kt_pack8(w, lo, hi);
    *reinterpret_cast<uint4_t*>(kt + kt_off(r0 + q * 8, n, N)) = lo;
    *reinterpret_cast<uint4_t*>(kt + kt_off(r0 + q * 8, n + 1, N)) = hi;
  }
}

__device__ __forceinline__ int tr_head_ld(int w) { return w + 16; }

__global__ __launch_bounds__(HNW * 64) void tr_head_kernel(TrHeadArgs a) {
  extern __shared__ __attribute__((aligned(16))) bf16_t lds[];
  const int nhb = static_cast<int>(gridDim.x) - a.nsample;
  if (static_cast<int>(blockIdx.x) >= nhb) {
    tr_sample_block<HNW * 64>(a.smp, blockIdx.x - nhb, reinterpret_cast<int32_t*>(lds));
    return;
  }
  const uint32_t blk = blockIdx.x;
  TR_STAMP(a.prof, blk, 0);
  const int Hin2 = a.Hin2, H = a.H, E = a.E, C = a.C;
  const int lda = tr_head_ld(Hin2), ldh = tr_head_ld(H), ldc = tr_head_ld(C);
  bf16_t* Aa = lds;
  bf16_t* Ah = Aa + HB * lda;
  bf16_t* Gb = Ah + HB * ldh;
  bf16_t* Dl = Gb + HB * ldh;
  bf16_t* Ly = Dl + HB * ldc;
  __shared__ int lab_s[HB];
  __shared__ float red_s[HNW][4];
  const int64_t r0 = static_cast<int64_t>(blockIdx.x) * HB;
  const int wave = threadIdx.x >> 6, lane = threadIdx.x & 63;
  const int lr = lane & 15, lg = lane >> 4;
  constexpr int NT = HNW * 64;

  if (a.label_mode < 2) {
    if (threadIdx.x < HB) {
      const int32_t root = a.roots[r0 + threadIdx.x];
      lab_s[threadIdx.x] = a.label_mode == 0 ? static_cast<int>(static_cast<const int16_t*>(a.labels)[root])
                                             : static_cast<const int32_t*>(a.labels)[root];
    }
  } else {
    const bf16_t* L = static_cast<const bf16_t*>(a.labels);
    const int cpl = C >> 3;
    for (int it = threadIdx.x; it < HB * cpl; it += NT) {
      const int r = it / cpl, c = it - r * cpl;
      const int64_t root = a.roots[r0 + r];
      *reinterpret_cast<uint4_t*>(Ly + r * C + c * 8) = *reinterpret_cast<const uint4_t*>(L + root * C + c * 8);
    }
  }
  const int nl = C >> 4, ne = E >> 4, nh = H >> 4;
  const int ne1 = (HNW - nl) > 0 ? ((HNW - nl) < ne ? (HNW - nl) : ne) : 0;
  const int n1 = nl + ne1, n2 = nh + ne + (ne - ne1);
  auto job1 = [&](int j, const bf16_t*& Bf, int& cc) {
    if (j < nl) {
      Bf = a.Wc;
      cc = j * 16;
    } else {
      Bf = a.Wfc;
      cc = (j - nl) * 16;
    }
  };
  auto job2 = [&](int j, const bf16_t*& Bf, int& cc, int& K) {
    if (j < nh) {
      Bf = a.WcT;
      cc = j * 16;
      K = C;
    } else if (j < nh + ne) {
      Bf = a.WoutT;
      cc = (j - nh) * 16;
      K = C;
    } else {
      Bf = a.Wfc;
      cc = (ne1 + j - nh - ne) * 16;
      K = H;
    }
  };

  uint4_t pre[TR_KC];
  tr_prefetch(a.W, wave * 16, H, Hin2, lane, pre);
  const int cpa = Hin2 >> 3;
  for (int it = threadIdx.x; it < HB * cpa; it += NT) {
    const int r = it / cpa, c = it - r * cpa;
    *reinterpret_cast<uint4_t*>(Aa + sw_off(r, c * 8, lda)) =
        *reinterpret_cast<const uint4_t*>(a.A + (r0 + r) * Hin2 + c * 8);
  }
  __syncthreads();
  TR_STAMP(a.prof, blk, 1);
  tr_lds_to_kt(Aa, lda, Hin2, r0, a.A_kt);
  for (int cc = wave * 16; cc < H; cc += HNW * 16) {
    float4_t acc[HFM][1];
    tl_zero(acc);
    tr_gemm(Aa, lda, a.W, cc, Hin2, acc, lane, pre);
    if (cc + HNW * 16 < H) tr_prefetch(a.W, cc + HNW * 16, H, Hin2, lane, pre);
#pragma unroll
    for (int m = 0; m < HFM; ++m)
#pragma unroll
      for (int j = 0; j < 4; ++j) Ah[sw_off(m * 16 + lg * 4 + j, cc + lr, ldh)] = f2bf(fmaxf(acc[m][0][j], 0.f));
  }
  if (wave < n1) {
    const bf16_t* Bf;
    int cc;
    job1(wave, Bf, cc);
    tr_prefetch(Bf, cc, 1 << 30, H, lane, pre);
  }
  __syncthreads();
  TR_STAMP(a.prof, blk, 2);
  tr_lds_to_kt(Ah, ldh, H, r0, a.h_kt);

  float lsum = 0.f;
  int tp = 0, fp = 0, fn = 0;
  for (int j = wave; j < n1; j += HNW) {
    const bf16_t* Bf;
    int cc;
    job1(j, Bf, cc);
    float4_t acc[HFM][1];
    tl_zero(acc);
    tr_gemm(Ah, ldh, Bf, cc, H, acc, lane, pre);
    const int col = cc + lr;
    if (j < nl) {
      const bool valid = col < a.C_real;
      const float bias = a.bc[col];
#pragma unroll
      for (int m = 0; m < HFM; ++m) {
        float d[4];
#pragma unroll
        for (int jj = 0; jj < 4; ++jj) {
          const int row = m * 16 + lg * 4 + jj;
          const float xv = acc[m][0][jj] + bias;
          const float y = a.label_mode < 2 ? ((lab_s[row] == col) ? 1.f : 0.f) : bf2f(Ly[row * C + col]);
          const float p = 1.f / (1.f + __expf(-xv));
          if (valid) {
            lsum += fmaxf(xv, 0.f) - xv * y + log1pf(__expf(-fabsf(xv)));
            const bool pred = xv >= 0.f, pos = y > 0.5f;
            tp += pred && pos;
            fp += pred && !pos;
            fn += !pred && pos;
          }
          d[jj] = valid ? bf2f(f2bf((p - y) * a.inv_scale)) : 0.f;
          Dl[sw_off(row, col, ldc)] = f2bf(d[jj]);
        }
        kt_store4(a.dlog_kt, r0 + m * 16 + lg * 4, col, C, d[0], d[1], d[2], d[3]);
      }
    } else {
      const float b = a.bfc[col];
#pragma unroll
      for (int m = 0; m < HFM; ++m)
        kt_store4(a.emb_kt, r0 + m * 16 + lg * 4, col, E, acc[m][0][0] + b, acc[m][0][1] + b, acc[m][0][2] + b,
                  acc[m][0][3] + b);
    }
    if (j + HNW < n1) {
      const bf16_t* Bn;
      int cn;
      job1(j + HNW, Bn, cn);
      tr_prefetch(Bn, cn, 1 << 30, H, lane, pre);
    }
  }
  {
    lsum = wave_sum(lsum);
    tp = wave_sum_i(tp);
    fp = wave_sum_i(fp);
    fn = wave_sum_i(fn);
    if (lane == 0) {
      red_s[wave][0] = lsum;
      red_s[wave][1] = static_cast<float>(tp);
      red_s[wave][2] = static_cast<float>(fp);
      red_s[wave][3] = static_cast<float>(fn);
    }
  }
  if (wave < n2) {
// ... 116 lines not shown
  {
    const int nc = H1 >> 4, nj = NTILE * nc;
    if (wave < nj) tr_prefetch(pr_tower(a, wave / nc).W1, (wave % nc) * 16, H1, H0x2, lane, pre);
    for (int j = wave; j < nj; j += HNW) {
      const int t = j / nc, cs = (j - t * nc) * 16;
      float4_t acc[HFM][1];
      tl_zero(acc);
      tr_gemm(Aa + 16 * t * lda, lda, pr_tower(a, t).W1, cs, H0x2, acc, lane, pre);
      if (j + HNW < nj) tr_prefetch(pr_tower(a, (j + HNW) / nc).W1, ((j + HNW) % nc) * 16, H1, H0x2, lane, pre);
      float v[4];
#pragma unroll
      for (int jj = 0; jj < 4; ++jj) {
        v[jj] = fmaxf(acc[0][0][jj], 0.f);
        Hh[sw_off(16 * t + lg * 4 + jj, cs + lr, ldh)] = f2bf(v[jj]);
      }
      kt_store4(pr_tower(a, t).h_kt, pr_row0(a, b, t) + lg * 4, cs + lr, H1, bf2f(f2bf(v[0])), bf2f(f2bf(v[1])),
                bf2f(f2bf(v[2])), bf2f(f2bf(v[3])));
    }
  }
  __syncthreads();
  {
    const int nc = E >> 4, nj = NTILE * nc;
    if (wave < nj) tr_prefetch(pr_tower(a, wave / nc).Wfc, (wave % nc) * 16, E, H1, lane, pre);
    for (int j = wave; j < nj; j += HNW) {
      const int t = j / nc, cs = (j - t * nc) * 16;
      float4_t acc[HFM][1];
      tl_zero(acc);
      tr_gemm(Hh + 16 * t * ldh, ldh, pr_tower(a, t).Wfc, cs, H1, acc, lane, pre);
      if (j + HNW < nj) tr_prefetch(pr_tower(a, (j + HNW) / nc).Wfc, ((j + HNW) % nc) * 16, E, H1, lane, pre);
      const float bias = pr_tower(a, t).bfc[cs + lr];
#pragma unroll
      for (int jj = 0; jj < 4; ++jj) Ef[(16 * t + lg * 4 + jj) * E + cs + lr] = acc[0][0][jj] + bias;
    }
  }
  __syncthreads();
  {
    const int i = wave;
    const int K = a.K;
    float l[16], g[16];
    const float* es = Ef + i * E;
#pragma unroll
    for (int k = 0; k < 16; ++k) {
      l[k] = 0.f;
      if (k > K) continue;
      const int row = k == 0 ? 16 + i : 32 + i * K + (k - 1);
      float d = 0.f;
      for (int c = lane; c < E; c += 64) d += es[c] * Ef[row * E + c];
      l[k] = wave_sum(d);
    }
    float loss = 0.f, gsum = 0.f;
    int beat = 0;
#pragma unroll
    for (int k = 0; k < 16; ++k) {
      g[k] = 0.f;
      if (k > K) continue;
      const float x = l[k];
      loss += fmaxf(x, 0.f) + log1pf(__expf(-fabsf(x))) - (k == 0 ? x : 0.f);
      g[k] = (1.f / (1.f + __expf(-x)) - (k == 0 ? 1.f : 0.f)) * a.inv_n;
      gsum += g[k];
      if (k > 0 && x >= l[0]) ++beat;
    }
    if (lane == 0) {
      red_s[i][0] = loss * a.inv_n;
      red_s[i][1] = 1.f / static_cast<float>(1 + beat);
    }
    for (int c = lane; c < E; c += 64) {
      const float ev = es[c];
      float de = 0.f;
#pragma unroll
      for (int k = 0; k < 16; ++k) {
        if (k > K) continue;
        const int row = k == 0 ? 16 + i : 32 + i * K + (k - 1);
        de += g[k] * Ef[row * E + c];
        Dd[sw_off(row, c, lde)] = f2bf(g[k] * ev);
      }
      Dd[sw_off(i, c, lde)] = f2bf(de);
      ps[i * E + c] = de;
      ps[(16 + i) * E + c] = gsum * ev;
    }
  }
  __syncthreads();
  for (int t = 0; t < NTILE; ++t) tr_lds_to_kt(Dd + 16 * t * lde, lde, E, pr_row0(a, b, t), pr_tower(a, t).de_kt);
  for (int c = threadIdx.x; c < 2 * E; c += NT) {
    const int tw = c >= E, col = c - tw * E;
    float v = 0.f;
    for (int w = 0; w < 16; ++w) v += ps[(tw * 16 + w) * E + col];
    (tw ? a.c : a.s).dbfc_part[static_cast<int64_t>(b) * E + col] = v;
  }
  if (threadIdx.x < 4) {
    float v = 0.f;
    if (threadIdx.x < 2)
      for (int w = 0; w < 16; ++w) v += red_s[w][threadIdx.x];
    a.head_part[b * 4 + threadIdx.x] = v;
  }
  {
    const int nc = H1 >> 4, nj = NTILE * nc;
    if (wave < nj) tr_prefetch(pr_tower(a, wave / nc).WfcT, (wave % nc) * 16, H1, E, lane, pre);
    for (int j = wave; j < nj; j += HNW) {
      const int t = j / nc, cs = (j - t * nc) * 16;
      float4_t acc[HFM][1];
      tl_zero(acc);
      tr_gemm(Dd + 16 * t * lde, lde, pr_tower(a, t).WfcT, cs, E, acc, lane, pre);
      if (j + HNW < nj) tr_prefetch(pr_tower(a, (j + HNW) / nc).WfcT, ((j + HNW) % nc) * 16, H1, E, lane, pre);
      float v[4];
#pragma unroll
      for (int jj = 0; jj < 4; ++jj) {
        const int row = 16 * t + lg * 4 + jj;
        v[jj] = bf2f(f2bf(bf_pos(Hh[sw_off(row, cs + lr, ldh)]) ? acc[0][0][jj] : 0.f));
        Gg[sw_off(row, cs + lr, ldh)] = f2bf(v[jj]);
      }
      kt_store4(pr_tower(a, t).g_kt, pr_row0(a, b, t) + lg * 4, cs + lr, H1, v[0], v[1], v[2], v[3]);
    }
  }
  __syncthreads();
  {
    const int nc = H0x2 >> 4, nj = NTILE * nc;
    if (wave < nj) tr_prefetch(pr_tower(a, wave / nc).W1T, (wave % nc) * 16, H0x2, H1, lane, pre);
    for (int j = wave; j < nj; j += HNW) {
      const int t = j / nc, cs = (j - t * nc) * 16;
      float4_t acc[HFM][1];
      tl_zero(acc);
      tr_gemm(Gg + 16 * t * ldh, ldh, pr_tower(a, t).W1T, cs, H1, acc, lane, pre);
      if (j + HNW < nj) tr_prefetch(pr_tower(a, (j + HNW) / nc).W1T, ((j + HNW) % nc) * 16, H0x2, H1, lane, pre);
      float* out = pr_tower(a, t).dA1;
      const int64_t r0 = pr_row0(a, b, t);
#pragma unroll
      for (int jj = 0; jj < 4; ++jj) out[(r0 + lg * 4 + jj) * H0x2 + cs + lr] = acc[0][0][jj];
    }
  }
}

}

using namespace euler_hip;

extern "C" {

size_t eh_tr_head_lds(int Hin2, int H, int E, int C, int label_mode) {
  (void)E;
  size_t el = static_cast<size_t>(HB) * ((Hin2 + 16) + 2 * (H + 16) + (C + 16));
  if (label_mode == 2) el += static_cast<size_t>(HB) * C;
  return el * sizeof(bf16_t);
}

hipError_t eh_tr_head(const TrHeadArgs* a, int64_t B, hipStream_t s) {
  if (!a->A || !a->W || !a->Wfc || !a->WfcT || !a->Wout || !a->WoutT || !a->Wc || !a->WcT || !a->bc || !a->bfc ||
      !a->roots || !a->labels ||
      !a->A_kt || !a->h_kt || !a->emb_kt || !a->dlog_kt || !a->demb_kt || !a->g_kt || !a->dbfc_part || !a->head_part ||
      (a->dA && !a->WT))
    return hipErrorInvalidValue;
  if (B % 32 != 0 || a->H % 16 != 0 || a->E % 32 != 0 || a->C % 32 != 0 || a->Hin2 % 32 != 0 ||
      a->C_real > a->C || a->C_real <= 0)
    return hipErrorInvalidValue;
  const size_t lds = eh_tr_head_lds(a->Hin2, a->H, a->E, a->C, a->label_mode);
  if (lds > 160 * 1024 - 64) return hipErrorInvalidValue;
  EULER_HIP_CHECK(hipFuncSetAttribute(reinterpret_cast<const void*>(tr_head_kernel),
                                      hipFuncAttributeMaxDynamicSharedMemorySize, static_cast<int>(lds)));
  if (a->nsample > 0 && (!tr_sample_ok(a->smp, kTrHeadSampleRows, a->nsample) || a->smp.roots == a->roots))
    return hipErrorInvalidValue;
  hipLaunchKernelGGL(tr_head_kernel, dim3(static_cast<uint32_t>(B / HB + a->nsample)), dim3(HNW * 64), lds, s, *a);
  return hipGetLastError();
}

size_t eh_tr_pair_head_lds(int K, int H0x2, int H1, int E) {
  const size_t rows = 16 * static_cast<size_t>(2 + K);
  const size_t abytes = rows * (H0x2 + 16) * 2, ebytes = rows * E * 4, gbytes = rows * (H1 + 16) * 2;
  const size_t region = std::max(std::max(abytes, ebytes), gbytes);
  return region + rows * (H1 + 16) * 2 + rows * (E + 16) * 2 + 2 * 16 * static_cast<size_t>(E) * 4;
}

hipError_t eh_tr_pair_head(const TrPairHeadArgs* a, hipStream_t s) {
  if (a->B <= 0 || a->B % 16 != 0 || a->K < 1 || a->K > 15 || a->H0x2 % 32 != 0 || a->H1 % 32 != 0 ||
      a->E % 32 != 0 || a->E > 1024)
    return hipErrorInvalidValue;
  const TrPairTower* tw[2] = {&a->s, &a->c};
  for (const TrPairTower* t : tw)
    if (!t->A1 || !t->W1 || !t->W1T || !t->Wfc || !t->WfcT || !t->bfc || !t->A1_kt || !t->h_kt || !t->de_kt ||
        !t->g_kt || !t->dA1 || !t->dbfc_part)
      return hipErrorInvalidValue;
  if (!a->head_part) return hipErrorInvalidValue;
  const size_t lds = eh_tr_pair_head_lds(a->K, a->H0x2, a->H1, a->E);
  if (lds > 160 * 1024 - 256) return hipErrorInvalidValue;
  EULER_HIP_CHECK(hipFuncSetAttribute(reinterpret_cast<const void*>(tr_pair_head_kernel),
                                      hipFuncAttributeMaxDynamicSharedMemorySize, static_cast<int>(lds)));
  hipLaunchKernelGGL(tr_pair_head_kernel, dim3(static_cast<uint32_t>(a->B / 16)), dim3(HNW * 64), lds, s, *a);
  return hipGetLastError();
}

}
```

### euler_amd/csrc/hip/tree_plan.h

```cpp
#pragma once
#include "hip/tree_args.h"

namespace euler_hip {

inline bool tr_sample_ok(const TrSampleArgs& a, int rows_per_block, int64_t nblocks) {
  if (!a.g.indptr || !a.g.nbr || !a.g.cumw || !a.g.prob || !a.g.alias || !a.tr.rng || !a.roots || !a.nodes || !a.leaf)
    return false;
  if (a.FL < 1 || a.lv < 0 || a.lv > 2 || rows_per_block < 1) return false;
  return nblocks == (a.M + rows_per_block - 1) / rows_per_block;
}

inline void tr_plan_stored(TrDwProb& p, int64_t target, int64_t min_kps, bool fold) {
  const int64_t MB = p.MB;
  const int64_t tiles = ((p.P + 63) / 64) * ((p.Q + 63) / 64);
  int64_t kps = (MB * tiles + target - 1) / target;
  if (kps < min_kps) kps = min_kps;
  if (kps > MB) kps = MB;
  const int64_t slabs = (MB + kps - 1) / kps;
  p.kps = static_cast<int32_t>(kps);
  p.F = fold && slabs <= kTrFoldMax ? static_cast<int32_t>(slabs) : 0;
  p.S = p.F ? 1 : static_cast<int32_t>(slabs);
}

constexpr int kTrRouteP = 64, kTrRouteQ = 128;
inline int32_t tr_route_tiles_q(const TrDwProb& p) { return (p.Q + kTrRouteQ - 1) / kTrRouteQ; }
inline int32_t tr_route_tiles(const TrDwProb& p) { return (p.P / kTrRouteP) * tr_route_tiles_q(p); }

inline bool tr_plan_routed(TrDwProb& p, int64_t target) {
  if (p.P < kTrRouteP || p.P % kTrRouteP != 0 || p.Q < 1 || p.MB < 1 || target < 1) return false;
  const int64_t MB = p.MB, tiles = tr_route_tiles(p);
  int64_t S = (target + tiles - 1) / tiles;
  S = (S + 7) / 8 * 8;
  if (S > (MB + 7) / 8 * 8) S = (MB + 7) / 8 * 8;
  p.kps = static_cast<int32_t>((MB + S - 1) / S);
  p.S = static_cast<int32_t>(S);
  return true;
}

inline int tr_seg_groups(const TrSeg& s) { return s.cols == 0 && s.S > 16 ? 4 : 1; }
inline int tr_seg_blocks(const TrSeg& s) {
  if (s.cols > 0) return (s.rows / 8) * (s.cols / 32);
  const int64_t per = 256 / tr_seg_groups(s);
  return static_cast<int>((s.n + per - 1) / per);
}

inline int tr_seg_layout(TrSeg* seg, int n, bool fill) {
  if (n < 1 || n > kTrMaxSegs) return -1;
  int blk = 0;
  for (int k = 0; k < n; ++k) {
    TrSeg& g = seg[k];
    if (fill) {
      g.blk0 = blk;
      g.sgrp = tr_seg_groups(g);
    }
    if (!g.part || g.S < 1 || g.blk0 != blk) return -1;
    if (g.cols > 0) {
      if (g.rows % 8 != 0 || g.cols % 32 != 0 || static_cast<int64_t>(g.rows) * g.cols != g.n) return -1;
    } else if (g.cols < 0 || g.sh || g.shT || g.sgrp != tr_seg_groups(g)) {
      return -1;
    }
    blk += tr_seg_blocks(g);
  }
  return blk;
}

struct TrDwGrid {
  int32_t ndw = 0;
  int32_t ntrail = 0;
  int32_t rtiles[2] = {0, 0};
};

inline bool tr_dw_layout(TrDwLaunch& L, TrDwGrid& grid) {
  grid = TrDwGrid{};
  TrDwProbs& pr = L.plain;
  if (pr.n < 0 || pr.n > kTrMaxProbs || L.nroute < 0 || L.nroute > 2) return false;
  L.rwg[0] = 0;
  for (int r = 0; r < L.nroute; ++r) {
    TrDwProb& p = L.route[r];
    if (!p.route || !p.dA || !p.mask || !p.X || !p.part) return false;
    if (p.P % kTrRouteP != 0 || p.Q % 32 != 0 || p.MB < 1 || p.kps < 1 || p.logPg < 3) return false;
    if (p.S % 8 != 0 || static_cast<int64_t>(p.S) * p.kps < p.MB) return false;
    p.tiles_q = tr_route_tiles_q(p);
    p.ntiles = tr_route_tiles(p);
    p.wg0 = 0;
    grid.rtiles[r] = p.ntiles;
    L.rwg[r + 1] = L.rwg[r] + p.ntiles * p.S;
  }
  int wg = 0;
  for (int i = 0; i < pr.n; ++i) {
    TrDwProb& p = pr.p[i];
    if (p.P % 32 != 0 || p.Q % 32 != 0 || p.MB < 1 || p.kps < 1) return false;
    if (p.route || !p.G || !p.X || !p.part) return false;
    if (p.F < 0 || p.F > kTrFoldMax || p.S < 1) return false;
    if (p.F > 0 && p.S != 1) return false;
    if (static_cast<int64_t>(p.F > 0 ? p.F : p.S) * p.kps < p.MB) return false;
    const int t = p.F > 0 ? 32 : 64;
    p.tiles_q = (p.Q + t - 1) / t;
    p.ntiles = ((p.P + t - 1) / t) * p.tiles_q;
    p.wg0 = wg;
    wg += p.ntiles * p.S;
  }
  L.ndw = grid.ndw = L.rwg[L.nroute] + wg;
  if (grid.ndw == 0 || !L.fuse) return true;
  TrDwOpt& o = L.opt;
  if (L.fuse != 1 || !o.p || !o.m || !o.v || !o.c.step || !o.c.loss_acc || !o.c.loss_out || !o.c.head_part ||
      o.c.nhead < 1 || !o.sync || o.timeout < 1 || o.rseg0 < 0 || o.rseg0 + L.nroute != o.nseg)
    return false;
  for (int i = 0; i < pr.n; ++i)
    if (pr.p[i].F < 1 || o.fseg[i].off < 0 || o.fseg[i].off % 4 != 0 || (o.fseg[i].shT && !o.fseg[i].sh)) return false;
  const int trail = tr_seg_layout(o.seg, o.nseg, false);
  if (trail < 0 || trail != o.nblk) return false;
  int line = 2;
  for (int k = 0; k < o.nseg; ++k) {
    const TrSeg& g = o.seg[k];
    if (k < o.rseg0) {
      if (g.cols != 0) return false;
      continue;
    }
    const TrDwProb& p = L.route[k - o.rseg0];
    if (g.cols < 1 || g.part != p.part || g.S != p.S || g.rows != p.P || g.cols != p.Q || (g.shT && !g.sh))
      return false;
    o.cnt0[k - o.rseg0] = line;
    line += p.ntiles;
  }
  if (line != o.nsync) return false;
  grid.ntrail = trail;
  return true;
}

inline bool tr_dw_fuse(const TrDwLaunch& L, const TrOptArgs& o, TrDwOpt& f) {
  f = TrDwOpt{};
  const TrSeg* rseg[2] = {nullptr, nullptr};
  bool pseg[kTrMaxProbs] = {};
  int nvec = 0;
  for (int k = 0; k < o.nseg; ++k) {
    const TrSeg& g = o.seg[k];
    if (g.cols == 0) {
      f.seg[nvec++] = g;
      continue;
    }
    bool found = false;
    for (int r = 0; r < L.nroute && !found; ++r)
      if (L.route[r].part == g.part && !rseg[r]) {
        rseg[r] = &g;
        found = true;
      }
    for (int i = 0; i < L.plain.n && !found; ++i) {
      const TrDwProb& p = L.plain.p[i];
      if (p.part != g.part || pseg[i]) continue;
      if (p.F < 1 || g.S != 1 || g.rows != p.P || g.cols != p.Q || g.off % 4 != 0) return false;
      f.fseg[i] = TrFoldSeg{g.off, g.sh, g.shT};
      pseg[i] = true;
      found = true;
    }
    if (!found) return false;
  }
  for (int i = 0; i < L.plain.n; ++i)
    if (!pseg[i]) return false;
  f.rseg0 = nvec;
  f.nseg = nvec + L.nroute;
  if (f.nseg > kTrMaxSegs) return false;
  f.nsync = 2;
  for (int r = 0; r < L.nroute; ++r) {
    if (!rseg[r]) return false;
    f.seg[nvec + r] = *rseg[r];
    f.nsync += L.route[r].ntiles;
  }
  f.nblk = tr_seg_layout(f.seg, f.nseg, true);
  if (f.nblk < 0) return false;
  f.p = o.p;
  f.m = o.m;
  f.v = o.v;
  f.c = o.c;
  f.timeout = kTrFuseWaitTicks;
  return o.c.nhead > 0;
}

}
```

### euler_amd/models/sage_trainer.py

```python
from __future__ import annotations

import math
import os

import numpy as np
import torch
import torch.nn.functional as F

from euler_amd.ops import mp_ops
from euler_amd.ops._native import hip
from euler_amd.models._tower_ops import env_plan_keys
from euler_amd.models.captured import new_graph

__all__ = ["SageTrainer", "sage_param_names"]

_OPT_KIND = {"adam": 0, "adagrad": 1, "sgd": 2, "momentum": 3}


def _ceil(x: int, m: int) -> int:
    return -(-int(x) // m) * m


def _slot(f: int) -> int:
    p = 4
    while (1 << p) < f + 1:
        p += 1
    return p


def sage_param_names(num_layers: int):
    names = []
    for k in range(num_layers):
        names += [f"gnn.convs.{k}.self_fc.weight", f"gnn.convs.{k}.neigh_fc.weight"]
    return names + ["gnn.fc.weight", "gnn.fc.bias", "out_fc.weight"]


def _xavier(shape, gen):
    fan_out, fan_in = shape
    a = math.sqrt(6.0 / (fan_in + fan_out))
    return (torch.rand(shape, generator=gen, dtype=torch.float64) * 2 - 1).mul_(a).float()


_SAMPLE_IN_OPT = os.environ.get("EULER_AMD_SAMPLE_IN", "head") == "opt"
_PIPELINE = os.environ.get("EULER_AMD_PIPELINE", "0") == "1"


class SageTrainer:
    def __init__(self, graph, batch_size, fanouts, dims, label_dim, features=None, labels=None, metapath=None,
                 add_self_loops=False, optimizer="adam", learning_rate=0.01, betas=(0.9, 0.999), eps=1e-8,
                 weight_decay=0.0, init=None, init_seed=0, keep_samples=True, grad_buckets=1, feature_shard=None,
                 feature_dim=None):
        self.graph = graph
        self.fshard = feature_shard
        self.device = graph.device
        self.B = int(batch_size)
        self.fanouts = [int(f) for f in fanouts]
        self.L = len(self.fanouts)
        if not 1 <= self.L <= 3:
            raise ValueError("1 to 3 hops are supported")
        dims = [int(d) for d in dims]
        if len(dims) != self.L + 1:
            raise ValueError("dims = conv widths (one per hop) + the fc width (reference dims[:-1] / dims[-1])")
        if self.B % 32:
            raise ValueError("batch_size must be a multiple of 32")
        self.conv_dims, self.E = dims[:-1], dims[-1]
        if grad_buckets not in (1, 2):
            raise ValueError("grad_buckets must be 1 or 2")
        self.n_buckets = int(grad_buckets)
        self.C = int(label_dim)
        self.include_self = bool(add_self_loops)
        self.opt_name = optimizer
        if optimizer not in _OPT_KIND:
            raise ValueError(f"optimizer must be one of {sorted(_OPT_KIND)}")
        self.lr, self.betas, self.eps, self.wd = float(learning_rate), tuple(betas), float(eps), float(weight_decay)
        if optimizer == "momentum" and betas == (0.9, 0.999):
            self.betas = (0.9, 0.0)
        if optimizer == "adagrad" and eps == 1e-8:
            self.eps = 1e-10
        feats = features if features is not None else graph.features
        if feature_shard is not None:
            feats = feature_shard.shard
            if feats.shape[1] % 16 or feats.dtype not in (torch.bfloat16, torch.float32):
                raise ValueError("sharded features must be bf16 / fp32 with a width padded to 16")
            if feature_dim is not None and _ceil(int(feature_dim), 16) != feats.shape[1]:
                raise ValueError(f"feature_dim {feature_dim} does not pad to the shard's {feats.shape[1]} columns")
        labs = labels if labels is not None else graph.labels
        if feats is None or labs is None:
            raise ValueError("features and labels are required (or a graph built with from_engine)")
        self.D = int(feature_dim) if feature_dim is not None else int(feats.shape[1])
        masks = metapath if metapath is not None else [None] * self.L
        if len(masks) != self.L:
            raise ValueError("one metapath entry (edge types) per hop")
        self.masks = [graph._mask(m) for m in masks]

        self.Dp = _ceil(self.D, 16)
        self.Hp = [_ceil(h, 64) for h in self.conv_dims]
        self.Ep, self.Cp = _ceil(self.E, 32), _ceil(self.C, 32)
        self.logP = [0] + [_slot(self.fanouts[k - 1]) for k in range(1, self.L)]
        self.M = [self.B]
        for k in range(1, self.L):
            self.M.append(self.M[-1] << self.logP[k])
        self.on_gpu = self.device.type == "cuda"

        self.features = self._pad_cols(feats, self.Dp, feats.dtype if feats.dtype in (torch.bfloat16,
                                                                                  torch.float32) else torch.float32)
        self.label_mode, self.labels = self._label_table(labs)

        self._shapes = self._logical_shapes()
        logical = self._init_logical(init, init_seed)
        self._build_flat()
        self.keep_samples = keep_samples
        self.step_count = 0
        if self.on_gpu:
            self._alloc_gpu()
            self.load_logical(logical)
        else:
            self._cpu_params = {k: v.clone().to(self.device).requires_grad_(True) for k, v in logical.items()}
            self._cpu_m = {k: torch.zeros_like(v) for k, v in logical.items()}
            self._cpu_v = {k: torch.full_like(v, 0.1 if optimizer == "adagrad" else 0.0) for k, v in
                           logical.items()}
            self._cpu_loss = torch.zeros(())
            self.pipelined, self._gathered = False, False
            self._cpu_counts = [0, 0, 0]
            self._cpu_samples = None
        self._graph_exec = None

    @classmethod
    def from_model(cls, model, graph, batch_size, optimizer="adam", learning_rate=0.01, **kw):
        from euler_amd.convolution.convs import SAGEConv
        from euler_amd.dataflow.dataflows import SageDataFlow
        import euler_amd.ops.graph_api as ge

        gnn = model.gnn
        if not all(isinstance(c, SAGEConv) for c in gnn.convs) or not isinstance(gnn.sampler, SageDataFlow):
            raise ValueError("the device path trains SAGEConv + SageDataFlow models (SupervisedGraphSage)")
        dims = [c.self_fc.out_features for c in gnn.convs] + [gnn.fc.out_features]
        metapath = []
        for m in gnn.sampler.metapath:
            ids = None if m is None else [int(t) for t in np.asarray(ge.get_edge_type_id(m)).reshape(-1)]
            metapath.append(None if ids is None or any(t < 0 for t in ids) else ids)
        return cls(graph, batch_size, gnn.sampler.fanouts, dims, model.label_dim, metapath=metapath,
                   add_self_loops=bool(getattr(gnn.sampler, "add_self_loops", False)), optimizer=optimizer,
                   learning_rate=learning_rate, init=model, **kw)

    def _pad_cols(self, t, width, dtype):
        t = t.to(self.device)
        if t.shape[1] == width and t.dtype == dtype and t.is_contiguous():
            return t
        out = torch.zeros((t.shape[0], width), dtype=dtype, device=self.device)
        out[:, : t.shape[1]] = t.to(dtype)
        return out

    def _label_table(self, labs):
        labs = labs.to(self.device)
        if labs.dim() == 1 or (labs.dim() == 2 and labs.shape[1] == 1 and not labs.is_floating_point()):
            labs = labs.reshape(-1)
            if labs.dtype == torch.int16:
                return 0, labs.contiguous()
            return 1, labs.to(torch.int32).contiguous()
        if labs.shape[1] != self.C:
            raise ValueError(f"label table has {labs.shape[1]} columns, label_dim is {self.C}")
        self._labels_dense = labs.float()
        return 2, self._pad_cols(labs, self.Cp, torch.bfloat16)

    def _logical_shapes(self):
        shapes = {}
        hin = self.D
        for k, h in enumerate(self.conv_dims):
            shapes[f"gnn.convs.{k}.self_fc.weight"] = (h, hin)
            shapes[f"gnn.convs.{k}.neigh_fc.weight"] = (h, hin)
            hin = h
        shapes["gnn.fc.weight"] = (self.E, hin)
        shapes["gnn.fc.bias"] = (self.E,)
        shapes["out_fc.weight"] = (self.C, self.E)
        return shapes

    def _init_logical(self, init, seed):
        if init is not None and not isinstance(init, dict):
            sd = init.state_dict()
            init = {k: sd[k] for k in self._shapes if k in sd}
        gen = torch.Generator().manual_seed(int(seed))
        out = {}
        for k, shp in self._shapes.items():
            if init is not None and k in init:
                v = torch.as_tensor(init[k]).detach().float().cpu()
                if tuple(v.shape) != tuple(shp):
                    raise ValueError(f"{k}: shape {tuple(v.shape)} != {shp}")
                out[k] = v.clone()
            elif k.endswith("bias"):
                out[k] = torch.zeros(shp)
            else:
                out[k] = _xavier(shp, gen)
        return out

    def _build_flat(self):
        sizes = []
        hin = self.Dp
        for h in self.Hp:
            sizes.append(h * 2 * hin)
            hin = h
        sizes += [self.Ep * hin, self.Ep, self.Cp * self.Ep]
        self.offsets = [0]
        for s in sizes:
            self.offsets.append(self.offsets[-1] + s)

    def _flat_views(self, flat):
        o = self.offsets
        views = []
        hin = self.Dp
        for k, h in enumerate(self.Hp):
            views.append(flat[o[k]:o[k + 1]].view(h, 2 * hin))
            hin = h
        L = self.L
        views.append(flat[o[L]:o[L + 1]].view(self.Ep, hin))
        views.append(flat[o[L + 1]:o[L + 2]])
        views.append(flat[o[L + 2]:o[L + 3]].view(self.Cp, self.Ep))
        return views

    def _pack(self, logical, flat):
        flat.zero_()
        v = self._flat_views(flat)
        hin, hinp = self.D, self.Dp
        for k, h in enumerate(self.conv_dims):
            v[k][:h, :hin] = logical[f"gnn.convs.{k}.self_fc.weight"].to(flat)
            v[k][:h, hinp:hinp + hin] = logical[f"gnn.convs.{k}.neigh_fc.weight"].to(flat)
            hin, hinp = h, self.Hp[k]
        L = self.L
        v[L][: self.E, :hin] = logical["gnn.fc.weight"].to(flat)
        v[L + 1][: self.E] = logical["gnn.fc.bias"].to(flat)
        v[L + 2][: self.C, : self.E] = logical["out_fc.weight"].to(flat)

    def _unpack(self, flat):
        v = self._flat_views(flat)
        out = {}
        hin, hinp = self.D, self.Dp
        for k, h in enumerate(self.conv_dims):
            out[f"gnn.convs.{k}.self_fc.weight"] = v[k][:h, :hin].clone()
            out[f"gnn.convs.{k}.neigh_fc.weight"] = v[k][:h, hinp:hinp + hin].clone()
            hin, hinp = h, self.Hp[k]
        L = self.L
        out["gnn.fc.weight"] = v[L][: self.E, :hin].clone()
        out["gnn.fc.bias"] = v[L + 1][: self.E].clone()
        out["out_fc.weight"] = v[L + 2][: self.C, : self.E].clone()
        return out

    def _alloc_gpu(self):
        dev, B, L = self.device, self.B, self.L
        bf = dict(dtype=torch.bfloat16, device=dev)
        f32 = dict(dtype=torch.float32, device=dev)
        i32 = dict(dtype=torch.int32, device=dev)
        n = self.offsets[-1]
        self.flat = torch.zeros(n, **f32)
        self.grad = torch.zeros(n, **f32)
        self.m = torch.zeros(n, **f32)
        self.v = torch.zeros(n, **f32)
        self._step = torch.zeros(1, dtype=torch.int64, device=dev)
        self.loss_acc = torch.zeros(1, **f32)
        self.loss_out = torch.zeros(1, **f32)
        self.counts = torch.zeros(3, **i32)
        if self.opt_name == "adagrad":
            self.v.fill_(0.1)
        g = self.graph
        d = {"L": L, "B": B, "F": [0] + self.fanouts, "logP": self.logP[:L] if L > 1 else [0],
             "masks": [0] + [int(m) & 0xFFFFFFFF for m in self.masks], "H": self.Hp, "D": self.Dp,
             "E": self.Ep, "C": self.Cp, "C_real": self.C, "include_self": int(self.include_self),
             "indptr": g.indptr, "nbr": g.nbr, "cumw": g.cumw, "num_types": g.num_types, "node_prob": g.node_prob,
             "node_alias": g.node_alias, "root_rows": g.root_rows, "rng": g.rng,
             "labels": self.labels, "label_mode": self.label_mode,
             "step": self._step, "flat": self.flat, "grad": self.grad, "m": self.m, "v": self.v,
             "label_rows": getattr(self, "_label_rows", None),
             "offsets": self.offsets, "loss_acc": self.loss_acc, "loss_out": self.loss_out, "counts": self.counts,
             "lr": self.lr, "beta1": self.betas[0], "beta2": self.betas[1], "eps": self.eps,
             "weight_decay": self.wd, "opt_kind": _OPT_KIND[self.opt_name]}
        env_plan_keys(d, "DW_TARGET_WG", "DW_MIN_KPS", "DW_ROUTE_WG", "FWD_BM", "DW_ROUTE_IMPL", "DW_FOLD",
                      "DW_OPT_FUSE")
        M_last = self.M[L - 1]
        FL = self.fanouts[-1]
        self.roots = torch.zeros(B, **i32)
        d["roots"] = self.roots
        self.nodes = torch.zeros(M_last, **i32)
        self.leaf = torch.zeros(M_last * FL, **i32)
        d["nodes"], d["leaf"] = self.nodes, self.leaf
        if self.fshard is None:
            d["features"] = self.features
            if _PIPELINE and L == 2:
                d["A0_rows"] = torch.empty(M_last * 2 * self.Dp, **bf)
        else:
            n = M_last * (1 + FL)
            self.fshard.alloc_cache(n)
            self._fpos = torch.full((n,), -1, **i32)
            d["fwd_features"] = self.fshard.cache
            d["fwd_nodes"], d["fwd_leaf"] = self._fpos[:M_last], self._fpos[M_last:]
        hin = [self.Dp] + self.Hp[:-1]
        for k in range(L):
            rows = self.M[L - 1 - k]
            d[f"A{k}_kt"] = torch.empty(rows * 2 * hin[k], **bf)
            if k >= 1 or L == 1:
                d[f"A{k}"] = torch.empty(rows * 2 * hin[k], **bf)
            if k < L - 1:
                d[f"mask{k}"] = torch.zeros((rows // 32) * self.Hp[k], **i32)
                d[f"dA{k + 1}"] = torch.empty(self.M[L - 2 - k] * 2 * self.Hp[k], **f32)
        H = self.Hp[-1]
        for name, cols in (("h_kt", H), ("emb_kt", self.Ep), ("dlog_kt", self.Cp), ("demb_kt", self.Ep),
                           ("g_kt", H)):
            d[name] = torch.empty(B * cols, **bf)
        views = self._flat_views(self.flat)
        for k in range(L):
            d[f"W{k}_sh"] = torch.empty(views[k].numel(), **bf)
            if k >= 1:
                d[f"W{k}_shT"] = torch.empty(views[k].numel(), **bf)
        for name, t in (("Wfc", views[L]), ("Wout", views[L + 2])):
            d[f"{name}_sh"] = torch.empty(t.numel(), **bf)
            d[f"{name}_shT"] = torch.empty(t.numel(), **bf)
        d["bfc"] = views[L + 1]
        self._buf = d
        self.plan = hip().TreePlan(d)
        self._dw_all = list(range(self.plan.num_problems()))
        self._primed = False
        self.pipelined = bool(self.plan.pipeline_ok())
        self._fused = bool(self.plan.fused()) and not _SAMPLE_IN_OPT and not self.pipelined
        self._gathered = False

    def load_logical(self, logical):
        if self.on_gpu:
            self._pack({k: torch.as_tensor(v) for k, v in logical.items()}, self.flat)
            self.refresh_shadows()
        else:
            self._param_version = getattr(self, "_param_version", 0) + 1
            with torch.no_grad():
                for k, v in logical.items():
                    self._cpu_params[k].copy_(torch.as_tensor(v).to(self._cpu_params[k]))

    def refresh_shadows(self):
        self._param_version = getattr(self, "_param_version", 0) + 1
        if self.on_gpu:
            self.plan.opt(3)

    def logical_params(self):
        if self.on_gpu:
            return self._unpack(self.flat.detach())
        return {k: v.detach().clone() for k, v in self._cpu_params.items()}

    def state_dict(self):
        return {k: v.cpu() for k, v in self.logical_params().items()}

    def write_to_model(self, model):
        sd = model.state_dict()
        with torch.no_grad():
            for k, v in self.logical_params().items():
                sd[k].copy_(v.to(sd[k]))

    def trainer_state(self):
        if self.on_gpu:
            m, v = self._unpack(self.m), self._unpack(self.v)
            step = int(self._step.item())
        else:
            m = {k: t.clone() for k, t in self._cpu_m.items()}
            v = {k: t.clone() for k, t in self._cpu_v.items()}
            step = self.step_count
        return {"m": {k: t.cpu() for k, t in m.items()}, "v": {k: t.cpu() for k, t in v.items()}, "step": step,
                "rng": self.graph.rng.detach().cpu().clone(), "optimizer": self.opt_name}

    def dp_state_tensors(self):
        if self.on_gpu:
            return [self.flat, self.m, self.v, self._step]
        return [t.data for t in self._cpu_params.values()] + list(self._cpu_m.values()) + list(self._cpu_v.values())

    def load_trainer_state(self, st):
        self.graph.rng.copy_(torch.as_tensor(st["rng"]).to(self.graph.rng))
        self.step_count = int(st["step"])
        self._primed = False
        self._gathered = False
        if self.on_gpu:
            self._pack({k: torch.as_tensor(t) for k, t in st["m"].items()}, self.m)
            self._pack({k: torch.as_tensor(t) for k, t in st["v"].items()}, self.v)
            self._step.fill_(int(st["step"]))
        else:
            for k in self._cpu_m:
                self._cpu_m[k].copy_(torch.as_tensor(st["m"][k]))
                self._cpu_v[k].copy_(torch.as_tensor(st["v"][k]))

    def _prime(self):
        if not self._primed:
            self.plan.sample()
            self._primed = True
            self._gathered = False

    def _fwd(self):
        if self.fshard is not None:
            self.fshard.exchange(torch.cat([self.nodes, self.leaf]), pos_out=self._fpos)
        self.plan.fwd()

    def forward_backward(self):
        p = self.plan
        self._prime()
        self._fwd()
        p.head()
        self._primed = False
        self._gathered = False
        p.bwd()
        p.dw(self._dw_all)
        p.opt(0)

    def optimizer_step(self, grad_scale: float = 1.0):
        self._param_version = getattr(self, "_param_version", 0) + 1
        self.plan.opt(1, float(grad_scale))

    def grad_buckets(self):
        o = self.offsets
        if self.n_buckets == 1 or self.L == 1:
            return [("all", 0, o[-1])]
        return [("head", o[self.L - 1], o[-1]), ("routed", 0, o[self.L - 1])]

    def fused(self, grad_sync=None) -> bool:
        return self.on_gpu and self._fused and grad_sync is None

    def fuse_error(self) -> int:
        return int(self.plan.fuse_error()) if self.on_gpu else 0

    def _check_fuse(self):
        if self.on_gpu and self._fused and self.plan.fuse_error():
            raise RuntimeError("a fused dW + optimizer launch timed out waiting for its routed blocks: "
                               "the parameters of that step are wrong")

    def step(self, grad_sync=None):
        self.step_count += 1
        if not self.on_gpu:
            return self._cpu_step(grad_sync)
        p = self.plan
        self._prime()
        if self.pipelined and self._gathered:
            p.fwd(None, True)
        else:
            self._fwd()
        smp_opt = _SAMPLE_IN_OPT and grad_sync is None
        p.head(None, not smp_opt)
        p.bwd()
        gat = self.pipelined
        if grad_sync is None and self._fused:
            p.dw(self._dw_all, None, True, 1.0)
        elif grad_sync is None:
            p.dw(self._dw_all)
            p.opt(2, 1.0, smp_opt, gat)
        elif len(self.grad_buckets()) == 1:
            p.dw(self._dw_all)
            p.opt(0, 1.0, False, gat)
            g = self.grad if getattr(self, "grad16", None) is None else self.grad16
            scale = grad_sync(g)
            p.opt(1, 1.0 if scale is None else float(scale))
        else:
            self._dist_backward(grad_sync, gat)
        self._primed = True
        self._gathered = gat

    def _dist_backward(self, grad_sync, gather=False):
        p = self.plan
        if not hasattr(self, "_comm_stream"):
            self._comm_stream = torch.cuda.Stream(device=self.device)
            nseg = self.L + 3
            self._segs_head = list(range(self.L - 1, nseg))
            self._segs_routed = list(range(0, self.L - 1))
        g = self.grad if getattr(self, "grad16", None) is None else self.grad16
        (_, a0, a1), (_, b0, b1) = self.grad_buckets()
        main, side = torch.cuda.current_stream(self.device), self._comm_stream
        side.wait_stream(main)
        with torch.cuda.stream(side):
            p.dw(p.problems(False))
            p.opt_segments(0, self._segs_head, True)
            scale = grad_sync(g[a0:a1])
        if self._segs_routed:
            p.dw(p.problems(True))
            p.opt_segments(0, self._segs_routed, False)
            side.wait_stream(main)
            with torch.cuda.stream(side):
                grad_sync(g[b0:b1])
        main.wait_stream(side)
        p.opt(1, 1.0 if scale is None else float(scale), False, gather)

    def plan_launches(self):
        p = self.plan
        out = [("sample", p.sample), ("fwd", self._fwd), ("head", p.head),
               ("head+sample", lambda: p.head(None, True))]
        if self.L == 3:
            out.append(("bwd", p.bwd))
        if self._fused:
            out.append(("dw+opt", lambda: p.dw(self._dw_all, None, True, 1.0)))
        else:
            out += [("dw", lambda: p.dw(self._dw_all)), ("opt", lambda: p.opt(2))]
        if self.pipelined:
            out += [("opt+gather", lambda: p.opt(2, 1.0, False, True)), ("fwd_gemm", lambda: p.fwd(None, True))]
        return out

    def capture(self, grad_sync=None, warmup: int = 2, steps: int = 1, extra_sizes=()):
        if not self.on_gpu:
            return None
        s = torch.cuda.Stream(device=self.device)
        s.wait_stream(torch.cuda.current_stream(self.device))
        with torch.cuda.stream(s):
            for _ in range(warmup):
                self.step(grad_sync)
        torch.cuda.current_stream(self.device).wait_stream(s)
        torch.cuda.synchronize(self.device)
        self._graphs = {}
        for k in sorted({1, int(steps)} | {int(e) for e in extra_sizes if int(e) > 0}, reverse=True):
            g = new_graph()
            with torch.cuda.graph(g, capture_error_mode="thread_local"):
                for _ in range(k):
                    self.step(grad_sync)
            self.step_count -= k
            self._graphs[k] = g
        self._graph_steps = int(steps)
        self._graph_exec = self._graphs[1]
        return self._graphs[int(steps)]

    def replay(self, n: int = 1):
        for _ in range(int(n)):
            self._graph_exec.replay()
        self.step_count += int(n)

    def replay_steps(self, n: int):
        left = int(n)
        for k in sorted(self._graphs, reverse=True):
            while left >= k:
                self._graphs[k].replay()
                left -= k
        self.step_count += int(n)

    def release_graphs(self):
        for g in getattr(self, "_graphs", {}).values():
            g.reset()
        self._graphs = {}
        self._graph_exec = None

    def set_grad_sync_dtype(self, dtype):
        if not self.on_gpu:
            self.set_grad_sync_dtype_cpu(dtype)
            return
        if dtype in (torch.bfloat16, "bf16", "bfloat16"):
            self.grad16 = torch.zeros(self.grad.numel(), dtype=torch.bfloat16, device=self.device)
            self.plan.set_grad16(self.grad16)
        else:
            self.grad16 = None
            self.plan.set_grad16(None)

    def use_grad_buffer(self, t: torch.Tensor):
        if not self.on_gpu:
            raise RuntimeError("use_grad_buffer: GPU trainers only")
        if t.dtype == torch.bfloat16:
            if getattr(self, "grad16", None) is None:
                raise ValueError("bf16 gradient buffer without set_grad_sync_dtype('bf16')")
            t.copy_(self.grad16)
            self.grad16 = t
            self.plan.set_grad16(t)
        else:
            t.copy_(self.grad)
            self.grad = t
            self.plan.set_grad(t)

    def set_learning_rate(self, lr: float):
        self.lr = float(lr)
        if self.on_gpu:
            self.plan.set_lr(self.lr)

    @property
    def loss(self) -> torch.Tensor:
        return self.loss_out if self.on_gpu else self._cpu_loss

    def metric(self) -> float:
        self._check_fuse()
        tp, fp, fn = (self.counts.tolist() if self.on_gpu else self._cpu_counts)
        return 2.0 * tp / max(2.0 * tp + fp + fn, 1e-12)

    def reset_metric(self):
        if self.on_gpu:
            self.counts.zero_()
        else:
            self._cpu_counts = [0, 0, 0]

    def samples(self):
        if self.on_gpu:
            if self._primed:
                raise RuntimeError("samples() describes the batch of the last forward_backward(); step() has "
                                   "already drawn the next batch into the sample buffers")
            return (self.roots.long(), self.nodes.long(), self.leaf.view(-1, self.fanouts[-1]).long())
        return self._cpu_samples

    def _cpu_sample(self):
        g, B = self.graph, self.B
        g.reseed_cpu()
        roots = g.sample_node(B).long()
        level = roots
        for k in range(1, self.L):
            f, P = self.fanouts[k - 1], 1 << self.logP[k]
            nb = g._sample_neighbor_cpu(level.int(), f, self.masks[k - 1], -1, False).long()
            slots = torch.full((level.numel(), P), -1, dtype=torch.int64)
            slots[:, :f] = nb
            slots[:, f] = level
            level = slots.reshape(-1)
        leaf = g._sample_neighbor_cpu(level.int(), self.fanouts[-1], self.masks[-1], -1, False).long()
        return roots, level, leaf

    def _labels_of(self, roots):
        if self.label_mode == 2:
            return self._labels_dense[roots.to(self._labels_dense.device)].float()
        y = torch.zeros((roots.numel(), self.C), dtype=torch.float32, device=self.labels.device)
        y.scatter_(1, self.labels[roots.to(self.labels.device)].long().view(-1, 1), 1.0)
        return y

    def _tree_of(self, roots):
        g = self.graph
        level = roots.long()
        types = lambda m: [t for t in range(g.num_types) if (m >> t) & 1]
        for k in range(1, self.L):
            f, P = self.fanouts[k - 1], 1 << self.logP[k]
            nb = g.sample_neighbor(level.int(), f, types(self.masks[k - 1]), -1, stream_id=7 + k).view(-1, f).long()
            slots = torch.full((level.numel(), P), -1, dtype=torch.int64, device=level.device)
            slots[:, :f] = nb
            slots[:, f] = level
            level = slots.reshape(-1)
        leaf = g.sample_neighbor(level.int(), self.fanouts[-1], types(self.masks[-1]), -1,
                                 stream_id=7 + self.L).view(-1, self.fanouts[-1]).long()
        g.advance()
        return level, leaf

    @torch.no_grad()
    def infer_logits(self, ids):
        rows = self.graph.rows_of(ids).to(self.graph.device)
        params = self.logical_params()
        nodes, leaf = self._tree_of(rows.clamp(min=0))
        emb = self.logical_embed(params, nodes, leaf)
        logits = emb @ params["out_fc.weight"].float().t().to(emb.device)
        return emb, logits, self._labels_of(rows.clamp(min=0)).to(emb.device)

    def infer_embed(self, ids):
        return self.infer_logits(ids)[0]

    def _unfm(self, sh, rows, cols):
        return sh.view(rows // 16, cols // 32, 4, 16, 8).permute(0, 3, 1, 2, 4).reshape(rows, cols)

    def _layerwise_weights(self):
        L = self.L
        if self.on_gpu:
            b = self._buf
# ... 216 lines not shown
```

Baseline: 15.63 million samples/s.

## Add optional head-kernel feature gather with double-buffered A0_kt; gate pipelining on env

Adds an optional mode where the head launch, after sampling leaves for the next step, also gathers their features into a second, alternately selected A0_kt buffer. The next forward then runs only its GEMM, and the dW kernel picks the matching buffer through a device-side selector. The goal is to hide the gather latency inside the head launch, at the cost of an extra feature buffer and more LDS use in the head kernel. This mode is off by default. The change also makes the pipelined forward depend on the EULER_AMD_PIPELINE variable (default off), so by default the plan now uses the fused dW+optimizer launch instead of the opt+gather pipeline.

```diff
diff --git a/euler_amd/_build.py b/euler_amd/_build.py
--- a/euler_amd/_build.py
+++ b/euler_amd/_build.py
@@ -166,10 +166,18 @@
 
 
 def build_plan_selftest() -> str:
+    return _build_plan_selftest("tree_plan_selftest")
+
+
+def build_head_gather_selftest() -> str:
+    return _build_plan_selftest("head_gather_selftest")
+
+
+def _build_plan_selftest(name: str) -> str:
     objdir = os.path.join(BUILD, "selftest_address")
     os.makedirs(objdir, exist_ok=True)
-    out = os.path.join(objdir, "tree_plan_selftest")
-    src = os.path.join(CSRC, "tests", "tree_plan_selftest.cc")
+    out = os.path.join(objdir, name)
+    src = os.path.join(CSRC, "tests", name + ".cc")
     hdir = os.path.join(CSRC, "hip")
     deps = [src, os.path.join(hdir, "tree_plan.h"), os.path.join(hdir, "tree_args.h"), __file__]
     if not os.path.exists(out) or os.path.getmtime(out) < _newest(deps):
diff --git a/euler_amd/csrc/hip/binding_tree.cpp b/euler_amd/csrc/hip/binding_tree.cpp
--- a/euler_amd/csrc/hip/binding_tree.cpp
+++ b/euler_amd/csrc/hip/binding_tree.cpp
@@ -8,6 +8,8 @@
 using namespace euler_hip;
 
 namespace {
+
+constexpr int64_t kHeadGatherDefault = 0;
 
 bool sync_debug() {
   static const bool on = [] {
@@ -175,10 +177,11 @@
     return w;
   }
 
-  void launch(const std::vector<int64_t>& which, c10::optional<torch::Tensor> prof, bool fuse, double grad_scale) {
+  void launch(const std::vector<int64_t>& which, c10::optional<torch::Tensor> prof, bool fuse, double grad_scale,
+              bool x_sel = false) {
     const c10::DeviceGuard g(pd_.device());
     TrDwGrid grid;
-    TrDwLaunch L = launch_of(which, fuse, grid);
+    TrDwLaunch L = launch_of(which, fuse, grid, x_sel);
     if (fuse) L.opt.c.grad_scale = static_cast<float>(grad_scale);
     if (prof.has_value()) {
       pd_.need(*prof, torch::kInt64, -1, "prof");
@@ -202,6 +205,12 @@
     return f;
   }
   void set_lr(double lr) { opt.c.lr = fopt_.c.lr = static_cast<float>(lr); }
+  void set_x_sel(const int32_t* sel, const uint16_t* b0, const uint16_t* b1) {
+    x_sel_ = sel;
+    x_buf_[0] = b0;
+    x_buf_[1] = b1;
+  }
+  int route_impl() const { return route_impl_; }
   void set_grad(torch::Tensor g, bool exact) {
     pd_.need(g, torch::kFloat32, exact ? opt.n : -1, "grad");
     TORCH_CHECK(g.numel() >= opt.n, "grad has ", g.numel(), " elements, fewer than the ", opt.n, " parameters");
@@ -216,15 +225,23 @@
   TrDwOpt fopt_{};
   torch::Tensor sync_;
   torch::Tensor grad_;
+  const int32_t* x_sel_ = nullptr;
+  const uint16_t* x_buf_[2] = {nullptr, nullptr};
 
   TrSeg& next_seg() {
     TORCH_CHECK(opt.nseg < kTrMaxSegs, pd_.name(), ": too many optimizer segments");
     return opt.seg[opt.nseg++] = TrSeg{};
   }
 
-  TrDwLaunch launch_of(const std::vector<int64_t>& which, bool fuse, TrDwGrid& grid) const {
+  TrDwLaunch launch_of(const std::vector<int64_t>& which, bool fuse, TrDwGrid& grid, bool x_sel = false) const {
     TrDwLaunch L{};
     L.route_impl = route_impl_;
+    if (x_sel) {
+      TORCH_CHECK(x_sel_, pd_.name(), ": this plan has no second A0_kt buffer to select");
+      L.x_sel = x_sel_;
+      L.x_buf[0] = x_buf_[0];
+      L.x_buf[1] = x_buf_[1];
+    }
     bool every = which.size() == probs.size();
     for (size_t k = 0; k < which.size(); ++k) {
       const int64_t i = which[k];
@@ -282,8 +299,13 @@
     build_head();
     build_dw();
     build_opt();
-    dw_.try_fuse(!pipeline_ok());
-  }
+    build_head_gather();
+    const int64_t pipe = has("pipeline") ? geti("pipeline") : 1;
+    TORCH_CHECK(pipe == 0 || pipe == 1, "TreePlan: pipeline must be 0 or 1");
+    dw_.try_fuse(!(pipeline_ok() && pipe == 1));
+  }
+
+  bool head_gather() const { return hg_; }
 
   bool fused() const { return dw_.fused(); }
   int64_t fuse_error() const { return dw_.fuse_error(); }
@@ -293,10 +315,12 @@
     tree_ok(eh_tr_sample(&sample_, cur_stream()), "tr_sample");
   }
 
-  void fwd(c10::optional<torch::Tensor> prof, bool gemm_only) {
+  void fwd(c10::optional<torch::Tensor> prof, bool gemm_only, bool head_gather) {
     const c10::DeviceGuard g(device());
     TORCH_CHECK(!gemm_only || pipeline_ok(), "TreePlan: no pipelined forward for this plan");
+    TORCH_CHECK(!head_gather || (gemm_only && hg_), "TreePlan: no head-gather forward for this plan");
     TrFwdArgs a0 = fwd0_;
+    if (head_gather) a0.kt_sel = kt_sel_;
     if (prof.has_value()) {
       need(*prof, torch::kInt64, (fwd0_.M / (gemm_only ? 64 : bm0_)) * 8, "prof");
       a0.prof = reinterpret_cast<long long*>(prof->data_ptr<int64_t>());
@@ -305,18 +329,32 @@
     if (L_ == 3) tree_ok(eh_tr_fwd(&fwd1_, 2, 0, bm1_, cur_stream()), "tr_fwd(inner)");
   }
 
-  void head(c10::optional<torch::Tensor> prof, bool with_sample) {
-    const c10::DeviceGuard g(device());
-    TrHeadArgs a = head_;
-    if (with_sample) {
+  void head(c10::optional<torch::Tensor> prof, bool with_sample, bool with_gather) {
+    const c10::DeviceGuard g(device());
+    TORCH_CHECK(!with_gather || (with_sample && hg_), "TreePlan: no head-gather launch for this plan");
+    TrHeadArgs a = with_gather ? head_gather_args() : head_;
+    if (with_sample && !with_gather) {
       a.smp = sample_;
       a.nsample = static_cast<int32_t>((sample_.M + kTrHeadSampleRows - 1) / kTrHeadSampleRows);
     }
     if (prof.has_value()) {
-      need(*prof, torch::kInt64, (B_ / kTrHeadRows) * 8, "prof");
+      need(*prof, torch::kInt64, -1, "prof");
+      const int64_t nh = B_ / kTrHeadRows;
+      TORCH_CHECK(prof->numel() == nh * 8 || prof->numel() == (nh + a.nsample) * 8,
+                  "prof: 8 stamps per head block, or per block of the grid");
       a.prof = reinterpret_cast<long long*>(prof->data_ptr<int64_t>());
-    }
-    tree_ok(eh_tr_head(&a, B_, cur_stream()), "tr_head");
+      a.prof_all = prof->numel() != nh * 8;
+    }
+    tree_ok(eh_tr_head(&a, B_, cur_stream()), with_gather ? "tr_head+gather" : "tr_head");
+  }
+  int64_t head_blocks(bool with_sample) const {
+    return B_ / kTrHeadRows + (with_sample ? (sample_.M + kTrHeadSampleRows - 1) / kTrHeadSampleRows : 0);
+  }
+  void head_prime() {
+    const c10::DeviceGuard g(device());
+    TORCH_CHECK(hg_, "TreePlan: no head-gather launch for this plan");
+    const TrHeadArgs a = head_gather_args();
+    tree_ok(eh_tr_head_prime(&a, cur_stream()), "tr_head(prime)");
   }
 
   void bwd() {
@@ -325,8 +363,9 @@
     tree_ok(eh_tr_bwd(&bwd1_, cur_stream()), "tr_bwd");
   }
 
-  void dw(std::vector<int64_t> which, c10::optional<torch::Tensor> prof, bool fuse, double grad_scale) {
-    dw_.launch(which, prof, fuse, grad_scale);
+  void dw(std::vector<int64_t> which, c10::optional<torch::Tensor> prof, bool fuse, double grad_scale, bool x_sel) {
+    TORCH_CHECK(!x_sel || hg_, "TreePlan: no second A0_kt buffer in this plan");
+    dw_.launch(which, prof, fuse, grad_scale, x_sel);
   }
   int64_t dw_blocks(bool fuse) const { return dw_.blocks(dw_.all(), fuse); }
 
@@ -415,6 +454,33 @@
   DwPlan dw_{*this};
   torch::Tensor roots_cur_;
   torch::Tensor g16_;
+  bool hg_ = false;
+  int32_t* kt_sel_ = nullptr;
+  uint16_t* kt2_ = nullptr;
+
+  TrHeadArgs head_gather_args() const {
+    TrHeadArgs a = head_;
+    a.smp = sample_;
+    a.nsample = static_cast<int32_t>((sample_.M + kTrHeadSampleRows - 1) / kTrHeadSampleRows);
+    a.gat = fwd0_;
+    a.gat.kt_sel = kt_sel_;
+    a.gat_kt[0] = fwd0_.a_kt;
+    a.gat_kt[1] = kt2_;
+    a.ngather = 1;
+    a.gat_fp32 = feat_fp32_;
+    return a;
+  }
+
+  void build_head_gather() {
+    const int64_t key = has("head_gather") ? geti("head_gather") : kHeadGatherDefault;
+    TORCH_CHECK(key == 0 || key == 1, "TreePlan: head_gather must be 0 or 1");
+    if (key == 0 || !pipeline_ok() || !has("A0_kt2") || dw_.route_impl() != 2) return;
+    kt2_ = bf("A0_kt2", fwd0_.M * 2 * D_);
+    kt_sel_ = zeros_ptr<int32_t>(1, torch::kInt32);
+    if (!tr_head_gather_ok(head_gather_args())) return;
+    dw_.set_x_sel(kt_sel_, fwd0_.a_kt, kt2_);
+    hg_ = true;
+  }
 
   int64_t Hin(int k) const { return k == 0 ? D_ : dims_[k - 1]; }
 
@@ -867,12 +933,17 @@
   py::class_<TreePlan>(m, "TreePlan")
       .def(py::init<py::dict>())
       .def("sample", &TreePlan::sample)
-      .def("fwd", &TreePlan::fwd, py::arg("prof") = py::none(), py::arg("gemm_only") = false)
+      .def("fwd", &TreePlan::fwd, py::arg("prof") = py::none(), py::arg("gemm_only") = false,
+           py::arg("head_gather") = false)
       .def("fwd_blocks", [](const TreePlan& t) { return t.fwd_blocks(); })
-      .def("head", &TreePlan::head, py::arg("prof") = py::none(), py::arg("with_sample") = false)
+      .def("head", &TreePlan::head, py::arg("prof") = py::none(), py::arg("with_sample") = false,
+           py::arg("with_gather") = false)
+      .def("head_prime", &TreePlan::head_prime)
+      .def("head_blocks", &TreePlan::head_blocks, py::arg("with_sample"))
+      .def("head_gather", &TreePlan::head_gather)
       .def("bwd", &TreePlan::bwd)
       .def("dw", &TreePlan::dw, py::arg("which"), py::arg("prof") = py::none(), py::arg("fuse") = false,
-           py::arg("grad_scale") = 1.0)
+           py::arg("grad_scale") = 1.0, py::arg("x_sel") = false)
       .def("fused", &TreePlan::fused)
       .def("dw_blocks", &TreePlan::dw_blocks, py::arg("fuse"))
       .def("fuse_error", &TreePlan::fuse_error)
diff --git a/euler_amd/csrc/hip/tree_args.h b/euler_amd/csrc/hip/tree_args.h
--- a/euler_amd/csrc/hip/tree_args.h
+++ b/euler_amd/csrc/hip/tree_args.h
@@ -8,6 +8,7 @@
 constexpr int kTrMaxSegs = 8;
 constexpr int kTrHeadRows = 16;
 constexpr int kTrHeadSampleRows = 256;
+constexpr int kTrHeadGatherRows = 128;
 
 struct TrGraph {
   const int64_t* indptr;
@@ -81,6 +82,7 @@
   TrCombArgs comb;
   int32_t ncomb;
   uint16_t* a_rows;
+  int32_t* kt_sel;
 };
 
 struct TrHeadArgs {
@@ -101,6 +103,10 @@
   long long* prof;
   TrSampleArgs smp;
   int32_t nsample;
+  TrFwdArgs gat;
+  uint16_t* gat_kt[2];
+  int32_t ngather, gat_fp32;
+  int32_t prof_all;
 };
 
 struct TrPairTower {
@@ -215,6 +221,8 @@
   long long* prof;
   int32_t ndw;
   int32_t fuse;
+  const int32_t* x_sel;
+  const uint16_t* x_buf[2];
   TrDwOpt opt;
 };
 
@@ -225,6 +233,7 @@
 hipError_t eh_tr_fwd(const euler_hip::TrFwdArgs* a, int mode, int feat_fp32, int bm, hipStream_t s);
 size_t eh_tr_gather32_lds(int D, int FL);
 hipError_t eh_tr_head(const euler_hip::TrHeadArgs* a, int64_t B, hipStream_t s);
+hipError_t eh_tr_head_prime(const euler_hip::TrHeadArgs* a, hipStream_t s);
 hipError_t eh_tr_bwd(const euler_hip::TrBwdArgs* a, hipStream_t s);
 hipError_t eh_tr_dw(euler_hip::TrDwLaunch* p, hipStream_t s);
 hipError_t eh_tr_opt(const euler_hip::TrOptArgs* a, int mode, hipStream_t s);
diff --git a/euler_amd/csrc/hip/tree_dev.h b/euler_amd/csrc/hip/tree_dev.h
--- a/euler_amd/csrc/hip/tree_dev.h
+++ b/euler_amd/csrc/hip/tree_dev.h
@@ -178,7 +178,8 @@
 constexpr int kTrSampleRows = 64;
 
 template <int NT>
-__device__ __forceinline__ void tr_sample_block(const TrSampleArgs& a, int blk, int32_t* node_s) {
+__device__ __forceinline__ void tr_sample_block(const TrSampleArgs& a, int blk, int32_t* node_s,
+                                                int32_t* leaf_s = nullptr) {
   constexpr int R = NT / 4;
   const int64_t row0 = static_cast<int64_t>(blk) * R;
   if (threadIdx.x < R) {
@@ -199,11 +200,13 @@
     const int64_t s = row0 + r;
     if (s >= a.M) break;
     const int32_t node = node_s[r];
-    a.leaf[s * a.FL + k] =
+    const int32_t v =
         node >= 0 ? tr_neighbor(a.g, node, a.mL,
                                 tr_rand(a.tr.rng, kTrStreamHop + a.hopL + a.tr.stream_off,
                                         static_cast<uint64_t>(s * a.FL + k)))
                   : -1;
+    a.leaf[s * a.FL + k] = v;
+    if (leaf_s) leaf_s[it] = v;
   }
 }
 
@@ -213,7 +216,7 @@
 
 __device__ __forceinline__ int f2_chunk(int r, int c) { return c ^ (r & 15); }
 
-template <typename FT, int BM, int NT>
+template <typename FT, int BM, int NT, int G = Feat8<FT>::kInFlight>
 __device__ __forceinline__ void f2_gather(const TrFwdArgs& a, bf16_t* At, const int32_t* node_s,
                                           const int32_t* leaf_s, int tid) {
   const int D = a.D, K2 = 2 * D;
@@ -221,7 +224,6 @@
   const int cpr = D >> 3;
   const int P = 1 << a.logPg, U = F2_SKIP_PAD ? a.Fg + 1 : P;
   const int nitems = (BM >> a.logPg) * U * cpr;
-  constexpr int G = Feat8<FT>::kInFlight;
   if (F2_SKIP_PAD && U < P) {
     const int pad = P - U, nch = K2 >> 3;
     for (int it = tid; it < (BM >> a.logPg) * pad * nch; it += NT) {
@@ -286,8 +288,7 @@
 }
 
 template <int BM, int NT>
-__device__ __forceinline__ void f2_kt(const TrFwdArgs& a, int64_t row0, const bf16_t* At, int tid) {
-  const int K2 = 2 * a.D;
+__device__ __forceinline__ void f2_kt_to(bf16_t* a_kt, int K2, int64_t row0, const bf16_t* At, int tid) {
   const int np = K2 >> 1;
   for (int it = tid; it < np * (BM / 8); it += NT) {
     const int q = it / np;
@@ -300,9 +301,13 @@
     }
     uint4_t lo, hi;
     kt_pack8(w, lo, hi);
-    *reinterpret_cast<uint4_t*>(a.a_kt + kt_off(row0 + q * 8, n, K2)) = lo;
-    *reinterpret_cast<uint4_t*>(a.a_kt + kt_off(row0 + q * 8, n + 1, K2)) = hi;
-  }
+    *reinterpret_cast<uint4_t*>(a_kt + kt_off(row0 + q * 8, n, K2)) = lo;
+    *reinterpret_cast<uint4_t*>(a_kt + kt_off(row0 + q * 8, n + 1, K2)) = hi;
+  }
+}
+template <int BM, int NT>
+__device__ __forceinline__ void f2_kt(const TrFwdArgs& a, int64_t row0, const bf16_t* At, int tid) {
+  f2_kt_to<BM, NT>(a.a_kt, 2 * a.D, row0, At, tid);
 }
 
 constexpr int kG32Rows = 32, kG32Threads = 256;
diff --git a/euler_amd/csrc/hip/tree_dw.hip b/euler_amd/csrc/hip/tree_dw.hip
--- a/euler_amd/csrc/hip/tree_dw.hip
+++ b/euler_amd/csrc/hip/tree_dw.hip
@@ -670,6 +670,7 @@
   }
 }
 
+template <bool XSEL>
 __global__ __launch_bounds__(256, 2) void tr_dw_all_kernel(TrDwLaunch a) {
   __shared__ __attribute__((aligned(16))) RouteLds gs;
   __shared__ uint4_t lut[256];
@@ -683,6 +684,9 @@
     const bool second = b >= a.rwg[1];
     TrDwProb pr = a.route[0];
     if (second) pr = a.route[1];
+    if constexpr (XSEL) {
+      if (!second) pr.X = a.x_sel[0] ? a.x_buf[0] : a.x_buf[1];
+    }
     uint32_t* ready = a.fuse ? a.opt.sync + static_cast<int64_t>(second ? a.opt.cnt0[1] : a.opt.cnt0[0]) * kTrSyncLine : nullptr;
     tr_dw_route_pipe_body(pr, second ? b - a.rwg[1] : b, gs, lut, second ? nullptr : a.prof, ready);
   } else if (a.nroute > 0 && b < a.rwg[1]) {
@@ -763,7 +767,8 @@
   TrDwGrid grid;
   if (!tr_dw_layout(*L, grid)) return hipErrorInvalidValue;
   if (grid.ndw == 0) return hipSuccess;
-  hipLaunchKernelGGL(tr_dw_all_kernel, dim3(static_cast<uint32_t>(grid.ndw + grid.ntrail)), dim3(256), 0, s, *L);
+  hipLaunchKernelGGL(L->x_sel ? tr_dw_all_kernel<true> : tr_dw_all_kernel<false>,
+                     dim3(static_cast<uint32_t>(grid.ndw + grid.ntrail)), dim3(256), 0, s, *L);
   return hipGetLastError();
 }
 
diff --git a/euler_amd/csrc/hip/tree_fwd.hip b/euler_amd/csrc/hip/tree_fwd.hip
--- a/euler_amd/csrc/hip/tree_fwd.hip
+++ b/euler_amd/csrc/hip/tree_fwd.hip
@@ -317,6 +317,7 @@
   if (tb == 0 && tid == 0) {
     if (a.step) a.step[0] += 1;
     a.rng[1] += 1;
+    if (GO && a.kt_sel) a.kt_sel[0] ^= 1;
   }
   for (int i = tb * NT + tid; i < a.B; i += ntb * NT) a.roots_cur[i] = a.roots_in[i];
   if constexpr (GO) {
diff --git a/euler_amd/csrc/hip/tree_head.hip b/euler_amd/csrc/hip/tree_head.hip
--- a/euler_amd/csrc/hip/tree_head.hip
+++ b/euler_amd/csrc/hip/tree_head.hip
@@ -61,11 +61,54 @@
 
 __device__ __forceinline__ int tr_head_ld(int w) { return w + 16; }
 
+#ifndef TR_HG_INFLIGHT_BF16
+#define TR_HG_INFLIGHT_BF16 5
+#endif
+#ifndef TR_HG_INFLIGHT_F32
+#define TR_HG_INFLIGHT_F32 3
+#endif
+template <typename FT>
+constexpr int kHgInFlight = sizeof(FT) == 2 ? TR_HG_INFLIGHT_BF16 : TR_HG_INFLIGHT_F32;
+
+template <typename FT>
+__device__ __forceinline__ void tr_sample_gather_block(const TrHeadArgs& a, int sb, bf16_t* lds) {
+  constexpr int NT = HNW * 64, R = kTrHeadSampleRows, SUB = kTrHeadGatherRows;
+  const int K2 = 2 * a.gat.D, FL = a.gat.FL, tid = threadIdx.x;
+  const uint32_t blk = blockIdx.x;
+  bf16_t* At = lds;
+  int32_t* node_s = reinterpret_cast<int32_t*>(lds + SUB * K2);
+  int32_t* leaf_s = node_s + R;
+  if (a.prof_all) TR_STAMP(a.prof, blk, 0);
+  tr_sample_block<NT>(a.smp, sb, node_s, leaf_s);
+  __syncthreads();
+  if (a.prof_all) TR_STAMP(a.prof, blk, 1);
+  bf16_t* kt = a.gat.kt_sel[0] ? a.gat_kt[1] : a.gat_kt[0];
+  const int cpr2 = K2 >> 3;
+#pragma unroll 1
+  for (int sub = 0; sub < R / SUB; ++sub) {
+    const int64_t row0 = static_cast<int64_t>(sb) * R + sub * SUB;
+    f2_gather<FT, SUB, NT, kHgInFlight<FT>>(a.gat, At, node_s + sub * SUB, leaf_s + sub * SUB * FL, tid);
+    __syncthreads();
+    f2_kt_to<SUB, NT>(kt, K2, row0, At, tid);
+    for (int it = tid; it < SUB * cpr2; it += NT) {
+      const int r = it / cpr2, c = it - r * cpr2;
+      *reinterpret_cast<uint4_t*>(a.gat.a_rows + (row0 + r) * K2 + c * 8) =
+          *reinterpret_cast<const uint4_t*>(At + r * K2 + f2_chunk(r, c) * 8);
+    }
+    __syncthreads();
+  }
+  if (a.prof_all) TR_STAMP(a.prof, blk, 2);
+}
+
+template <bool GATHER>
 __global__ __launch_bounds__(HNW * 64) void tr_head_kernel(TrHeadArgs a) {
   extern __shared__ __attribute__((aligned(16))) bf16_t lds[];
   const int nhb = static_cast<int>(gridDim.x) - a.nsample;
   if (static_cast<int>(blockIdx.x) >= nhb) {
-    tr_sample_block<HNW * 64>(a.smp, blockIdx.x - nhb, reinterpret_cast<int32_t*>(lds));
+    const int sb = static_cast<int>(blockIdx.x) - nhb;
+    if constexpr (!GATHER) tr_sample_block<HNW * 64>(a.smp, sb, reinterpret_cast<int32_t*>(lds));
+    else if (a.gat_fp32) tr_sample_gather_block<float>(a, sb, lds);
+    else tr_sample_gather_block<bf16_t>(a, sb, lds);
     return;
   }
   const uint32_t blk = blockIdx.x;
@@ -488,13 +531,27 @@
   if (B % 32 != 0 || a->H % 16 != 0 || a->E % 32 != 0 || a->C % 32 != 0 || a->Hin2 % 32 != 0 ||
       a->C_real > a->C || a->C_real <= 0)
     return hipErrorInvalidValue;
-  const size_t lds = eh_tr_head_lds(a->Hin2, a->H, a->E, a->C, a->label_mode);
-  if (lds > 160 * 1024 - 64) return hipErrorInvalidValue;
-  EULER_HIP_CHECK(hipFuncSetAttribute(reinterpret_cast<const void*>(tr_head_kernel),
-                                      hipFuncAttributeMaxDynamicSharedMemorySize, static_cast<int>(lds)));
+  size_t lds = eh_tr_head_lds(a->Hin2, a->H, a->E, a->C, a->label_mode);
+  if (lds > kTrHeadLdsMax) return hipErrorInvalidValue;
   if (a->nsample > 0 && (!tr_sample_ok(a->smp, kTrHeadSampleRows, a->nsample) || a->smp.roots == a->roots))
     return hipErrorInvalidValue;
-  hipLaunchKernelGGL(tr_head_kernel, dim3(static_cast<uint32_t>(B / HB + a->nsample)), dim3(HNW * 64), lds, s, *a);
+  if (a->ngather) {
+    if (!tr_head_gather_ok(*a)) return hipErrorInvalidValue;
+    lds = std::max(lds, tr_head_gather_lds(a->gat.D, a->gat.FL));
+  }
+  void (*const k)(TrHeadArgs) = a->ngather ? tr_head_kernel<true> : tr_head_kernel<false>;
+  EULER_HIP_CHECK(hipFuncSetAttribute(reinterpret_cast<const void*>(k), hipFuncAttributeMaxDynamicSharedMemorySize,
+                                      static_cast<int>(lds)));
+  hipLaunchKernelGGL(k, dim3(static_cast<uint32_t>(B / HB + a->nsample)), dim3(HNW * 64), lds, s, *a);
+  return hipGetLastError();
+}
+
+hipError_t eh_tr_head_prime(const TrHeadArgs* a, hipStream_t s) {
+  if (!tr_head_gather_ok(*a)) return hipErrorInvalidValue;
+  const size_t lds = tr_head_gather_lds(a->gat.D, a->gat.FL);
+  EULER_HIP_CHECK(hipFuncSetAttribute(reinterpret_cast<const void*>(tr_head_kernel<true>),
+                                      hipFuncAttributeMaxDynamicSharedMemorySize, static_cast<int>(lds)));
+  hipLaunchKernelGGL(tr_head_kernel<true>, dim3(static_cast<uint32_t>(a->nsample)), dim3(HNW * 64), lds, s, *a);
   return hipGetLastError();
 }
 
diff --git a/euler_amd/csrc/hip/tree_plan.h b/euler_amd/csrc/hip/tree_plan.h
--- a/euler_amd/csrc/hip/tree_plan.h
+++ b/euler_amd/csrc/hip/tree_plan.h
@@ -8,6 +8,21 @@
     return false;
   if (a.FL < 1 || a.lv < 0 || a.lv > 2 || rows_per_block < 1) return false;
   return nblocks == (a.M + rows_per_block - 1) / rows_per_block;
+}
+
+constexpr size_t kTrHeadLdsMax = 160 * 1024 - 64;
+inline size_t tr_head_gather_lds(int D, int FL) {
+  return static_cast<size_t>(kTrHeadGatherRows) * 2 * D * 2 + static_cast<size_t>(kTrHeadSampleRows) * (1 + FL) * 4;
+}
+inline bool tr_head_gather_ok(const TrHeadArgs& a) {
+  const TrFwdArgs& g = a.gat;
+  if (a.ngather != 1 || a.nsample < 1 || !tr_sample_ok(a.smp, kTrHeadSampleRows, a.nsample)) return false;
+  if (a.smp.roots == a.roots || a.smp.M % kTrHeadSampleRows != 0) return false;
+  if (g.nodes != a.smp.nodes || g.leaf != a.smp.leaf || g.M != a.smp.M || g.FL != a.smp.FL) return false;
+  if (!g.x || !g.a_rows || !g.kt_sel || !a.gat_kt[0] || !a.gat_kt[1] || a.gat_kt[0] == a.gat_kt[1]) return false;
+  if (a.gat_fp32 != 0 && a.gat_fp32 != 1) return false;
+  if (g.D < 64 || g.D % 64 != 0 || g.logPg < 2 || g.logPg > 5 || g.Fg < 0 || g.Fg >= (1 << g.logPg)) return false;
+  return tr_head_gather_lds(g.D, g.FL) <= kTrHeadLdsMax;
 }
 
 inline void tr_plan_stored(TrDwProb& p, int64_t target, int64_t min_kps, bool fold) {
@@ -74,6 +89,8 @@
   grid = TrDwGrid{};
   TrDwProbs& pr = L.plain;
   if (pr.n < 0 || pr.n > kTrMaxProbs || L.nroute < 0 || L.nroute > 2) return false;
+  if (L.x_sel && (L.nroute < 1 || L.route_impl != 2 || !L.x_buf[0] || !L.x_buf[1] || L.x_buf[0] == L.x_buf[1]))
+    return false;
   L.rwg[0] = 0;
   for (int r = 0; r < L.nroute; ++r) {
     TrDwProb& p = L.route[r];
diff --git a/euler_amd/models/sage_trainer.py b/euler_amd/models/sage_trainer.py
--- a/euler_amd/models/sage_trainer.py
+++ b/euler_amd/models/sage_trainer.py
@@ -43,6 +43,7 @@
 
 _SAMPLE_IN_OPT = os.environ.get("EULER_AMD_SAMPLE_IN", "head") == "opt"
 _PIPELINE = os.environ.get("EULER_AMD_PIPELINE", "0") == "1"
+_HEAD_GATHER = 0
 
 
 class SageTrainer:
@@ -121,6 +122,7 @@
                            logical.items()}
             self._cpu_loss = torch.zeros(())
             self.pipelined, self._gathered = False, False
+            self.head_gather, self._hgathered = False, False
             self._cpu_counts = [0, 0, 0]
             self._cpu_samples = None
         self._graph_exec = None
@@ -273,7 +275,11 @@
              "lr": self.lr, "beta1": self.betas[0], "beta2": self.betas[1], "eps": self.eps,
              "weight_decay": self.wd, "opt_kind": _OPT_KIND[self.opt_name]}
         env_plan_keys(d, "DW_TARGET_WG", "DW_MIN_KPS", "DW_ROUTE_WG", "FWD_BM", "DW_ROUTE_IMPL", "DW_FOLD",
-                      "DW_OPT_FUSE")
+                      "DW_OPT_FUSE", "HEAD_GATHER")
+        d.setdefault("head_gather", _HEAD_GATHER)
+        if L != 2 or self.fshard is not None or d["label_rows"] is not None:
+            d["head_gather"] = 0
+        d["pipeline"] = int(_PIPELINE)
         M_last = self.M[L - 1]
         FL = self.fanouts[-1]
         self.roots = torch.zeros(B, **i32)
@@ -283,8 +289,10 @@
         d["nodes"], d["leaf"] = self.nodes, self.leaf
         if self.fshard is None:
             d["features"] = self.features
-            if _PIPELINE and L == 2:
+            if (_PIPELINE or d["head_gather"]) and L == 2:
                 d["A0_rows"] = torch.empty(M_last * 2 * self.Dp, **bf)
+            if d["head_gather"] and L == 2:
+                d["A0_kt2"] = torch.empty(M_last * 2 * self.Dp, **bf)
         else:
             n = M_last * (1 + FL)
             self.fshard.alloc_cache(n)
@@ -317,7 +325,9 @@
         self.plan = hip().TreePlan(d)
         self._dw_all = list(range(self.plan.num_problems()))
         self._primed = False
-        self.pipelined = bool(self.plan.pipeline_ok())
+        self.pipelined = _PIPELINE and bool(self.plan.pipeline_ok())
+        self.head_gather = bool(self.plan.head_gather())
+        self._hgathered = False
         self._fused = bool(self.plan.fused()) and not _SAMPLE_IN_OPT and not self.pipelined
         self._gathered = False
 
@@ -371,6 +381,7 @@
         self.step_count = int(st["step"])
         self._primed = False
         self._gathered = False
+        self._hgathered = False
         if self.on_gpu:
             self._pack({k: torch.as_tensor(t) for k, t in st["m"].items()}, self.m)
             self._pack({k: torch.as_tensor(t) for k, t in st["v"].items()}, self.v)
@@ -385,6 +396,17 @@
             self.plan.sample()
             self._primed = True
             self._gathered = False
+            self._hgathered = False
+
+    def _hg_step(self, grad_sync=None) -> bool:
+        return self.on_gpu and self.head_gather and not self.pipelined and grad_sync is None
+
+    def _hg_fwd(self):
+        if not (self._primed and self._hgathered):
+            self.plan.head_prime()
+            self._primed = True
+            self._gathered = False
+        self.plan.fwd(None, True, True)
 
     def _fwd(self):
         if self.fshard is not None:
@@ -393,13 +415,18 @@
 
     def forward_backward(self):
         p = self.plan
-        self._prime()
-        self._fwd()
+        hg = self._hg_step()
+        if hg:
+            self._hg_fwd()
+        else:
+            self._prime()
+            self._fwd()
         p.head()
         self._primed = False
         self._gathered = False
+        self._hgathered = False
         p.bwd()
-        p.dw(self._dw_all)
+        p.dw(self._dw_all, None, False, 1.0, hg)
         p.opt(0)
 
     def optimizer_step(self, grad_scale: float = 1.0):
@@ -428,19 +455,23 @@
         if not self.on_gpu:
             return self._cpu_step(grad_sync)
         p = self.plan
-        self._prime()
-        if self.pipelined and self._gathered:
-            p.fwd(None, True)
-        else:
-            self._fwd()
-        smp_opt = _SAMPLE_IN_OPT and grad_sync is None
-        p.head(None, not smp_opt)
+        hg = self._hg_step(grad_sync)
+        if hg:
+            self._hg_fwd()
+        else:
+            self._prime()
+            if self.pipelined and self._gathered:
+                p.fwd(None, True)
+            else:
+                self._fwd()
+        smp_opt = _SAMPLE_IN_OPT and grad_sync is None and not hg
+        p.head(None, not smp_opt, hg)
         p.bwd()
         gat = self.pipelined
         if grad_sync is None and self._fused:
-            p.dw(self._dw_all, None, True, 1.0)
+            p.dw(self._dw_all, None, True, 1.0, hg)
         elif grad_sync is None:
-            p.dw(self._dw_all)
+            p.dw(self._dw_all, None, False, 1.0, hg)
             p.opt(2, 1.0, smp_opt, gat)
         elif len(self.grad_buckets()) == 1:
             p.dw(self._dw_all)
@@ -452,6 +483,7 @@
             self._dist_backward(grad_sync, gat)
         self._primed = True
         self._gathered = gat
+        self._hgathered = hg
 
     def _dist_backward(self, grad_sync, gather=False):
         p = self.plan
@@ -489,6 +521,10 @@
             out += [("dw", lambda: p.dw(self._dw_all)), ("opt", lambda: p.opt(2))]
         if self.pipelined:
             out += [("opt+gather", lambda: p.opt(2, 1.0, False, True)), ("fwd_gemm", lambda: p.fwd(None, True))]
+        if self.head_gather:
+            out.append(("head+sample+gather", lambda: p.head(None, True, True)))
+            if not self.pipelined:
+                out.append(("fwd_gemm", lambda: p.fwd(None, True, True)))
         return out
 
     def capture(self, grad_sync=None, warmup: int = 2, steps: int = 1, extra_sizes=()):
```

After: 15.61 million samples/s. No clear change (-0.1%).
